# JANUS-Institute/HallThrusterPEM

Measured on AMD Instinct MI355X. Metric: coupled PEM-v0 model evals/sec, higher is better.
Workload: dtype f64

## Files before the change

### hallthrusterpem_amd/_lib.py

```python
import ctypes as C
import importlib.util
import os
import threading
from pathlib import Path

PKG = Path(__file__).resolve().parent
LIB_PATH = PKG / 'libpem_hip.so'

PEM_OK, PEM_ERR_INVALID_ARG, PEM_ERR_HIP, PEM_ERR_NO_DEVICE = 0, 1, 2, 3
NANGLE = 91
FUSED_LATENT_MAX_RANK = 8
FUSED_SYSTEM_MAX_RECORDS = 1024
SYS_JION, SYS_VCC, SYS_T, SYS_UION = 0, 1, 2, 3
SWEEP_CATHODE, SWEEP_THRUSTER, SWEEP_PLUME = 0, 1, 2
DE_MAX_POP, DE_MAX_DIM = 1024, 16
DE_BEST1BIN, DE_RAND1BIN = 0, 1
CHAIN_TIME_BLOCK = 4096

_dp = C.c_void_p
_sz = C.c_size_t
_f8 = C.c_double

SIGNATURES = {
    'pem_version': (C.c_char_p, []),
    'pem_last_error': (C.c_char_p, []),
    'pem_device_count': (C.c_int, []),
    'pem_init': (C.c_int, [C.c_int]),
    'pem_synchronize': (C.c_int, [_dp]),
    'pem_set_lanes_per_sample': (C.c_int, [C.c_int]),
    'pem_angle_grid': (C.POINTER(C.c_double), []),
    'pem_persistent_grid': (C.c_int, [_sz, C.c_int, C.c_int, C.c_int, C.POINTER(_sz), C.POINTER(_sz)]),
    'pem_coupled_occupancy': (C.c_int, [C.c_int, C.POINTER(C.c_int), C.POINTER(C.c_int)]),
    'pem_cathode_f64_dev': (C.c_int, [_sz] + [_dp] * 6 + [_f8, _dp, _dp]),
    'pem_cathode_f64': (C.c_int, [_sz] + [_dp] * 6 + [_f8, _dp]),
    'pem_plume_f64_dev': (C.c_int, [_sz, C.c_int, _dp, _f8] + [_dp] * 10 + [_dp] * 4 + [_dp]),
    'pem_plume_f64': (C.c_int, [_sz, C.c_int, _dp, _f8] + [_dp] * 10 + [_dp] * 4),
    'pem_thruster_f64_dev': (C.c_int, [_sz] + [_dp] * 4 + [_dp] * 8 + [_dp]),
    'pem_thruster_f64': (C.c_int, [_sz] + [_dp] * 4 + [_dp] * 8),
    'pem_thruster_uion_f64_dev': (C.c_int, [_sz, _dp, _f8, _f8, C.c_int, _dp, _dp, _dp]),
    'pem_thruster_filter_f64_dev': (C.c_int, [_sz, C.c_int, _dp, _dp, _f8, C.c_int, _dp, _dp, _dp, _dp]),
    'pem_coupled_f64_dev': (C.c_int, [_sz, _f8, _f8] + [_dp] * 15 + [_dp] * 7 + [_dp]),
    'pem_coupled_f64': (C.c_int, [_sz, _f8, _f8] + [_dp] * 15 + [_dp] * 7),
    'pem_coupled_tiled_f64_dev': (C.c_int, [_sz, _f8, _f8, _dp] + [_dp] * 7 + [_dp]),
    'pem_coupled_mixed_dev': (C.c_int, [_sz, _f8, _f8] + [_dp] * 15 + [_dp] * 7 + [_dp]),
    'pem_coupled_loglik_f64_dev': (C.c_int, [_sz, _f8, _f8] + [_dp] * 15 + [C.c_int, C.c_int] + [_dp] * 4 + [_dp] * 5 + [_dp]),
    'pem_coupled_system_loglik_f64_dev': (C.c_int, [_sz, _f8, _f8] + [_dp] * 15 + [C.c_int, C.c_int, _dp, _dp, C.c_int, _dp, _f8, _f8, C.c_int]
                                          + [_dp] * 5 + [_dp]),
    'pem_coupled_system_predict_f64_dev': (C.c_int, [_sz, _f8, _f8] + [_dp] * 15 + [C.c_int, C.c_int, _dp, _dp, C.c_int, _dp, _f8, _f8, C.c_int]
                                           + [_dp] * 4 + [_sz, _dp, _dp]),
    'pem_predictive_inputs_f64_dev': (C.c_int, [_sz, C.c_int, C.c_uint64, C.c_uint64, C.c_uint32, _dp, _dp, _dp, _dp, _dp, _sz, C.c_int,
                                                _dp, C.c_uint32, _dp, _sz, _dp]),
    'pem_predictive_noise_f64_dev': (C.c_int, [_sz, C.c_int, _dp, _sz, _dp, C.c_uint64, C.c_uint64, C.c_uint32, _dp, _sz, _dp]),
    'pem_coupled_latent_f64_dev': (C.c_int, [_sz, _f8, _f8] + [_dp] * 15 + [C.c_int, C.c_int, _dp, _dp] + [_dp] * 4 + [_dp]),
    'pem_loglik_marginal_f64_dev': (C.c_int, [_sz, C.c_int, C.c_int, _dp, _dp, _dp, _f8, _f8, _dp, _dp, _dp]),
    'pem_log_prior_f64_dev': (C.c_int, [_sz, C.c_int, _dp, _dp, _dp, _dp, _dp, _dp, _dp, _dp]),
    'pem_jion_loglik_f64_dev': (C.c_int, [_sz, C.c_int, C.c_int] + [_dp] * 6 + [_dp]),
    'pem_svd_compress_f64_dev': (C.c_int, [_sz, C.c_int, C.c_int, C.c_int, _f8, _dp, _dp, _dp, _dp]),
    'pem_svd_reconstruct_f64_dev': (C.c_int, [_sz, C.c_int, C.c_int, C.c_int, _f8, _dp, _dp, _dp, _dp]),
    'pem_coupled_mc_f64_dev': (C.c_int, [_sz, C.c_uint64, C.c_uint64, C.c_uint32, C.c_int, _dp, _dp, _dp, _f8, _f8, _dp, _sz] + [_dp] * 7 + [_dp]),
    'pem_sparse_predict_f64_dev': (C.c_int, [_sz, C.c_int, C.c_int, _dp, _dp, _dp, C.c_int, _dp, _sz, _dp, _sz, C.c_int, C.c_int, _dp]),
    'pem_sparse_grid_values_f64_dev': (C.c_int, [_sz, C.c_int, C.c_int, _dp, _dp, _dp, C.c_int, _dp, _sz, _dp, _sz, C.c_int, C.c_int, _dp]),
    'pem_sparse_predict_field_f64_dev': (C.c_int, [_sz, C.c_int, C.c_int, _dp, _dp, _dp, C.c_int, _dp, _sz, _dp, _sz, C.c_int, C.c_int,
                                                   C.c_int, C.c_int, C.c_int, C.c_int, C.c_double, _dp, _dp, _dp]),
    'pem_sparse_predict_chain_f64_dev': (C.c_int, [_sz, C.c_int, C.c_int, C.c_int, _dp, _f8, _f8, _f8, _f8, _dp, _sz, _dp, _sz,
                                                   C.c_int, C.c_int, C.c_int, C.c_int, C.c_double, _dp, _dp, _dp]),
    'pem_key_minmax_f64_dev': (C.c_int, [_sz, C.c_int, _dp, _sz, _dp, _dp, _dp, _dp]),
    'pem_range_hist_f64_dev': (C.c_int, [_sz, C.c_int, _dp, _sz, C.c_int, _dp, _dp, C.c_int, _dp, _dp]),
    'pem_range_narrow_dev': (C.c_int, [C.c_int, C.c_int, _dp, _dp, _dp, _dp, _dp]),
    'pem_qsel_bins': (C.c_int, [C.c_int, C.c_int, C.POINTER(C.c_int), C.POINTER(C.c_int)]),
    'pem_qsel_minmax_f64_dev': (C.c_int, [_sz, C.c_int, _dp, _sz, _dp, _dp, _dp, _dp]),
    'pem_qsel_hist1_f64_dev': (C.c_int, [_sz, C.c_int, _dp, _sz, _dp, _dp, C.c_int, _dp, _dp]),
    'pem_qsel_decide1_dev': (C.c_int, [C.c_int, C.c_int, _dp, _dp, _dp, C.c_int, _dp, _dp, _dp, _dp, _dp]),
    'pem_qsel_hist2_f64_dev': (C.c_int, [_sz, C.c_int, _dp, _sz, _dp, _dp, C.c_int, _dp, C.c_int, C.c_int, _dp, _dp]),
    'pem_qsel_decide2_dev': (C.c_int, [C.c_int, C.c_int, _dp, _dp, C.c_int, _dp, _dp, _dp, _dp, _dp, _dp, _dp]),
    'pem_qsel_compact_f64_dev': (C.c_int, [_sz, C.c_int, _dp, _sz, _dp, _dp, C.c_int, _dp, _dp, _dp, C.c_int, C.c_int, C.c_uint32, _dp, _dp, _dp]),
    'pem_qsel_select_dev': (C.c_int, [C.c_int, C.c_int, C.c_int, C.c_uint32, _dp, _dp, _dp, _dp, _dp, _dp, _dp]),
    'pem_quantiles_f64_dev': (C.c_int, [_sz, C.c_int, _dp, _sz, C.c_int, _dp, _dp, _dp, _dp, _dp]),
    'pem_quantiles_strided_f64_dev': (C.c_int, [_sz, C.c_int, _dp, _sz, _sz, C.c_int, _dp, _dp, _dp, _dp, _dp]),
    'pem_quantiles_last_path': (C.c_int, []),
    'pem_coupled_mc_stats_f64_dev': (C.c_int, [_sz, C.c_uint64, C.c_uint64, C.c_uint32, _dp, _dp, _dp, C.c_double, C.c_double, _dp, _sz,
                                               _dp, _dp, _dp, _dp, _dp, _dp, _dp, _dp, C.c_int, _dp, _dp, _dp, _dp, _dp, _dp,
                                               C.c_int, C.c_int, C.c_double, _dp, _dp, _dp, _dp]),
    'pem_row_masks_f64_dev': (C.c_int, [_sz, C.c_int, _dp, _sz, _dp, _dp, _dp, _dp, _dp]),
    'pem_campaign_masks_f64_dev': (C.c_int, [_sz, C.c_int, _dp, _dp, C.c_int, C.c_int, C.c_int, C.c_double, _dp, _dp, _sz, _dp, _dp, C.c_int, _dp, _dp,
                                             C.c_int, _dp]),
    'pem_sobol_partial_f64_dev': (C.c_int, [_sz, C.c_int, _sz, _dp, _dp, _dp, _dp, C.c_int, _dp]),
    'pem_coupled_f32_dev': (C.c_int, [_sz, C.c_float, C.c_float, _dp, _sz, _dp, _sz, _dp, _dp]),
    'pem_saltelli_f32_dev': (C.c_int, [_sz, C.c_uint64, C.c_uint64, C.c_uint32, _dp, _dp, _dp, C.c_int, _dp, C.c_float, C.c_float, _dp, _dp, C.c_int, _dp]),
    'pem_saltelli_f64_dev': (C.c_int, [_sz, C.c_uint64, C.c_uint64, C.c_uint32, _dp, _dp, _dp, C.c_int, _dp, C.c_double, C.c_double, _dp, _dp, C.c_int, _dp]),
    'pem_sobol_sweep_f64_dev': (C.c_int, [C.c_int, _sz, C.c_uint64, C.c_uint64, C.c_int, _dp, _dp, _dp, _f8, _f8, _f8, _f8, _f8, C.c_int,
                                          _dp, _dp, _dp, _dp, C.c_int, _dp]),
    'pem_de_step_f64_dev': (C.c_int, [C.c_int, C.c_int, C.c_int, C.c_int, C.c_uint64, _f8, _f8, _f8, _f8, _f8, _dp, _dp, _dp, _dp, _dp, _dp,
                                      _dp, _dp, _dp, _dp, _dp, _sz, _dp]),
    'pem_sample_f64_dev': (C.c_int, [_sz, C.c_uint64, C.c_uint64, C.c_uint32, C.c_int, _dp, _dp, _dp, C.c_int, _dp, _sz, _dp]),
    'pem_sample_tiled_f64_dev': (C.c_int, [_sz, C.c_uint64, C.c_uint64, C.c_uint32, C.c_int, _dp, _dp, _dp, C.c_int, _dp, _dp]),
    'pem_sample_lhs_f64_dev': (C.c_int, [_sz, C.c_uint64, C.c_uint64, C.c_uint64, C.c_uint32, C.c_int, _dp, _dp, _dp, _dp, _sz, _dp]),
    'pem_chain_autocov_f64_dev': (C.c_int, [_sz, _sz, _sz, _dp] + [_sz] * 6 + [_dp, _dp, _dp, _sz, _dp]),
}


class SurrStage(C.Structure):
    _fields_ = [('index', _dp), ('coef', _dp), ('values', _dp), ('n_beta', C.c_int), ('n_out', C.c_int), ('max_active', C.c_int),
                ('max_level', C.c_int)]


_lib = None
_hip_runtime = None
_lock = threading.Lock()


class PemHipError(RuntimeError):

    def __init__(self, code, message):
        super().__init__(f'libpem_hip error {code}: {message}')
        self.code = code


def _share_torch_hip_runtime():
    if os.environ.get('PEM_HIP_RUNTIME', '').lower() == 'system':
        return None
    try:
        spec = importlib.util.find_spec('torch')
    except (ImportError, ValueError):
        spec = None
    if spec is None or not spec.submodule_search_locations:
        return None
    cand = Path(list(spec.submodule_search_locations)[0]) / 'lib' / 'libamdhip64.so'
    if not cand.exists():
        return None
    return C.CDLL(str(cand), mode=C.RTLD_GLOBAL)


def load():
    global _lib, _hip_runtime
    if _lib is not None:
        return _lib
    with _lock:
        if _lib is not None:
            return _lib
        path = Path(os.environ.get('PEM_HIP_LIB', LIB_PATH))
        if 'PEM_HIP_LIB' not in os.environ:
            from . import build as _build
            if _build.needs_build():
                if _build.have_hipcc():
                    _build.build()
                elif not path.exists():
                    raise RuntimeError('libpem_hip.so is missing and hipcc is not available to build it')
                else:
                    import warnings
                    warnings.warn('libpem_hip.so is older than its sources and hipcc is not available: loading the stale library')
        _hip_runtime = _share_torch_hip_runtime()
        lib = C.CDLL(str(path))
        for name, (res, args) in SIGNATURES.items():
            fn = getattr(lib, name)
            fn.restype = res
            fn.argtypes = args
        _lib = lib
    return _lib


def check(rc: int):
    if rc != PEM_OK:
        raise PemHipError(rc, load().pem_last_error().decode(errors='replace'))


# ... 29 lines not shown
```

### hallthrusterpem_amd/csrc/pem_kernels.hip

```cpp
#include <hip/hip_runtime.h>

#include <cmath>
#include <cstdarg>
#include <cstdint>
#include <cstdio>
#include <cstdlib>
#include <cstring>
#include <atomic>
#include <functional>
#include <future>
#include <mutex>
#include <string>
#include <thread>
#include <type_traits>

#include "pem_common.h"
#include "pem_math.h"
#include "pem_hip.h"
#include "pem_philox.h"
#include "pem_qfused.h"

#include "pem_model.h"

namespace {
// ... 2204 lines not shown

template <int JMODE>
int launch_count(const PlumeIO& io, const CoupledIO& cio, const McDesign& mc, int nq, hipStream_t st, unsigned* grid_only) {
    if (io.q.premask && nq <= 5) return launch_r1<4, true, JMODE, true, 5, true>(io, cio, st, mc, grid_only);
    if (nq <= 3) return launch_r1<4, true, JMODE, true, 3>(io, cio, st, mc, grid_only);
    if (nq <= 5) return launch_r1<4, true, JMODE, true, 5>(io, cio, st, mc, grid_only);
    return launch_r1<4, true, JMODE, true, 6>(io, cio, st, mc, grid_only);
}

}

namespace pem {

int launch_coupled_mc(const McLaunch& a, hipStream_t st) {
    if (a.n == 0) return PEM_OK;
    McDesign mc{};
    if (int rc = mc_design_of(a, &mc)) return rc;
    PlumeIO io{(long long)a.n, a.torr2pa, a.radius, nullptr, nullptr, nullptr, nullptr, nullptr, nullptr, nullptr, nullptr, nullptr, nullptr, a.j_ion, a.div_angle, a.T_c, a.invalid, nullptr};
    CoupledIO cio{nullptr, nullptr, nullptr, nullptr, nullptr, nullptr, nullptr, a.V_cc, a.I_B0, a.T};
    return a.j_ion ? launch_r1<4, true, 1, true>(io, cio, st, mc) : launch_r1<4, true, 0, true>(io, cio, st, mc);
}

static int count_launch(const McLaunch& a, const CountIO& c, bool store_profile, hipStream_t st, unsigned* grid_only) {
    McDesign mc{};
    if (int rc = mc_design_of(a, &mc)) return rc;
    PlumeIO io{(long long)a.n, a.torr2pa, a.radius, nullptr, nullptr, nullptr, nullptr, nullptr, nullptr, nullptr, nullptr, nullptr, nullptr, a.j_ion, a.div_angle, a.T_c, a.invalid, nullptr};
    io.q = c;
    CoupledIO cio{nullptr, nullptr, nullptr, nullptr, nullptr, nullptr, nullptr, a.V_cc, a.I_B0, a.T};
    return store_profile ? launch_count<4>(io, cio, mc, c.nq, st, grid_only) : launch_count<5>(io, cio, mc, c.nq, st, grid_only);
}

int coupled_count_waves(size_t n, int nq, bool store_profile, unsigned* waves) {
    McLaunch a{};
    a.n = n;
    for (int d = 0; d < 15; ++d) a.kind[d] = PEM_DIST_UNIFORM;
    CountIO c{};
    c.nq = nq;
    unsigned grid = 0;
    if (int rc = count_launch(a, c, store_profile, nullptr, &grid)) return rc;
    *waves = grid * WPB;
    return PEM_OK;
}

int launch_coupled_mc_count(const McLaunch& a, const CountIO& c, bool store_profile, hipStream_t st) {
    if (a.n == 0) return PEM_OK;
    if (c.nq < 1 || c.nq > 6 || !c.br || !c.below || !c.rec || !c.rec_count || !c.flags || c.cap == 0)
        return fail(PEM_ERR_INVALID_ARG, "counting launch: incomplete arguments");
    if (store_profile && !a.j_ion) return fail(PEM_ERR_INVALID_ARG, "counting launch: no profile array to store into");
    return count_launch(a, c, store_profile, st, nullptr);
}

}

extern "C" {

namespace {
struct ScalarJob {
    struct Stage {
        std::promise<int> go;
        std::future<int> gone;
        bool signalled = false;
        hipEvent_t ev = nullptr;
        Stage() : gone(go.get_future()) {}
        void signal(int v) {
            if (!signalled) {
                signalled = true;
                go.set_value(v);
            }
        }
        int launched(hipStream_t st) {
            if (signalled) return PEM_OK;
            HIP_TRY(hipEventRecord(ev, st));
            signal(1);
            return PEM_OK;
        }
        int await(hipStream_t side) {
            if (gone.get() != 1) return fail(PEM_ERR_HIP, "pem_coupled_mc_stats (scalar selection): given up");
            HIP_TRY(hipStreamWaitEvent(side, ev, 0));
            return PEM_OK;
        }
    };
    Stage pilot, full;
    Stage side;
    std::thread worker;
    std::function<void()> body;
    bool started = false;
    int rc = PEM_OK;
    std::string error;
    int start() {
        if (started) return PEM_OK;
        started = true;
        HIP_TRY(hipEventCreateWithFlags(&pilot.ev, hipEventDisableTiming));
        HIP_TRY(hipEventCreateWithFlags(&full.ev, hipEventDisableTiming));
        HIP_TRY(hipEventCreateWithFlags(&side.ev, hipEventDisableTiming));
        try {
            worker = std::thread(body);
        } catch (const std::exception& e) {
            return fail(PEM_ERR_HIP, "pem_coupled_mc_stats: could not start the scalar selection's thread: %s", e.what());
        }
        return PEM_OK;
    }
    int join() {
        pilot.signal(0);
        full.signal(0);
        if (worker.joinable()) worker.join();
        for (Stage* s : {&pilot, &full, &side}) {
            if (s->ev) (void)hipEventDestroy(s->ev);
            s->ev = nullptr;
        }
        return rc;
    }
    ~ScalarJob() { (void)join(); }
};

int side_stream(hipStream_t* out) {
    static std::mutex mu;
    static hipStream_t streams[64] = {};
    int dev = 0;
    HIP_TRY(hipGetDevice(&dev));
    if (dev < 0 || dev >= 64) return fail(PEM_ERR_INVALID_ARG, "device index out of range");
    std::lock_guard<std::mutex> lock(mu);
    if (!streams[dev]) HIP_TRY(hipStreamCreateWithFlags(&streams[dev], hipStreamNonBlocking));
    *out = streams[dev];
    return PEM_OK;
}

struct McProducer : pem::FusedProducer {
    pem::McLaunch a;
    bool store_profile;
    bool counted = false;
    ScalarJob* job = nullptr;
    int pilot(size_t rows, double* dst, hipStream_t st) override {
        pem::McLaunch p = a;
        p.n = rows;
        p.j_ion = dst;
        if (int rc = pem::launch_coupled_mc(p, st)) return rc;
        if (!job) return PEM_OK;
        if (int rc = job->start()) return rc;
        return job->pilot.launched(st);
    }
    int waves(int nq, unsigned* w) override { return pem::coupled_count_waves(a.n, nq, store_profile, w); }
    int count(const pem::CountIO& io, hipStream_t st) override {
        if (job && job->worker.joinable() && job->side.gone.get() == 1) HIP_TRY(hipStreamWaitEvent(st, job->side.ev, 0));
        if (int rc = pem::launch_coupled_mc_count(a, io, store_profile, st)) return rc;
        counted = true;
        return job ? job->full.launched(st) : PEM_OK;
    }
};
}

int pem_coupled_mc_stats_f64_dev(size_t n, uint64_t first_index, uint64_t seed, uint32_t stream_id, const int32_t* kind, const double* a,
                                 const double* b, double torr2pa, double radius, double* x_out, size_t ld, double* V_cc, double* I_B0,
                                 double* T, double* j_ion, double* pilot_rows, double* div_angle, double* T_c, uint8_t* invalid, int nq,
                                 const uint64_t* rank_prev, const uint64_t* rank_next, const double* gamma, double* q_out, double* q_scalars,
                                 int* fused_ok, int q25, int q75, double iqr_factor, uint8_t* row_certain, uint8_t* row_uncertain,
                                 int* premask_ok, pem_stream_t stream) {
    if (!kind || !a || !b || !V_cc || !div_angle || !T_c || !rank_prev || !rank_next || !gamma || !q_out || !fused_ok)
        return fail(PEM_ERR_INVALID_ARG, "pem_coupled_mc_stats: NULL array");
    if (!j_ion && !pilot_rows) return fail(PEM_ERR_INVALID_ARG, "pem_coupled_mc_stats: without a profile array, room for the pilot rows is needed");
    if (j_ion && !aligned16(j_ion)) return fail(PEM_ERR_INVALID_ARG, "pem_coupled_mc_stats: j_ion must be 16-byte aligned");
    if (pilot_rows && !aligned16(pilot_rows)) return fail(PEM_ERR_INVALID_ARG, "pem_coupled_mc_stats: pilot_rows must be 16-byte aligned");
    if (x_out && ld < n) return fail(PEM_ERR_INVALID_ARG, "pem_coupled_mc_stats: leading dimension smaller than n");
    if (nq < 1 || nq > PEM_QUANTILE_MAX_Q) return fail(PEM_ERR_INVALID_ARG, "pem_coupled_mc_stats: 1 <= nq <= %d", PEM_QUANTILE_MAX_Q);
    if (n < PEM_MC_STATS_MIN_N) return fail(PEM_ERR_INVALID_ARG, "pem_coupled_mc_stats: at least %d samples", PEM_MC_STATS_MIN_N);
    const ptrdiff_t qstride = div_angle - V_cc;
    if (q_scalars && (qstride < (ptrdiff_t)n || T_c - div_angle != qstride))
        return fail(PEM_ERR_INVALID_ARG, "pem_coupled_mc_stats: q_scalars needs V_cc, div_angle, T_c as equally spaced rows of one array");
    if (int rc = check_device()) return rc;
    hipStream_t st = static_cast<hipStream_t>(stream);
    ScalarJob job;
    McProducer prod;
    if (q_scalars) {
        int dev = 0;
        HIP_TRY(hipGetDevice(&dev));
        hipStream_t side = nullptr;
        if (int rc = side_stream(&side)) return rc;
        job.body = [&job, dev, side, n, nq, V_cc, qstride, rank_prev, rank_next, gamma, q_scalars]() {
            struct Release {
                ScalarJob& j;
                ~Release() { j.side.signal(0); }
            } release{job};
            auto note = [&job](int rc) {
                job.rc = rc;
                if (rc != PEM_OK) job.error = pem_last_error();
                return rc;
            };
            if (hipSetDevice(dev) != hipSuccess) {
                (void)note(fail(PEM_ERR_HIP, "pem_coupled_mc_stats (scalar selection): hipSetDevice failed"));
                return;
            }
            if (note(job.pilot.await(side))) return;
            pem::SidePlan plan;
            plan.ctx = &job;
            plan.before_full = [](void* ctx, hipStream_t st) {
                ScalarJob* j = static_cast<ScalarJob*>(ctx);
                if (j->side.launched(st)) j->side.signal(0);
                return j->full.await(st);
            };
            (void)note(pem::quantiles_side(n, 3, V_cc, 1, (size_t)qstride, nq, rank_prev, rank_next, gamma, q_scalars, side, &plan));
        };
        prod.job = &job;
    }
    prod.a.n = n;
    prod.a.first_index = first_index;
    prod.a.seed = seed;
    prod.a.stream_id = stream_id;
    for (int d = 0; d < 15; ++d) {
        prod.a.kind[d] = kind[d];
        prod.a.a[d] = a[d];
        prod.a.b[d] = b[d];
    }
    prod.a.torr2pa = torr2pa;
    prod.a.radius = radius;
    prod.a.x_out = x_out;
    prod.a.ld = ld;
    prod.a.V_cc = V_cc;
    prod.a.I_B0 = I_B0;
    prod.a.T = T;
    prod.a.j_ion = j_ion;
    prod.a.div_angle = div_angle;
    prod.a.T_c = T_c;
    prod.a.invalid = invalid;
    prod.store_profile = j_ion != nullptr;
    if (row_certain && row_uncertain && premask_ok) {
        prod.pm_q25 = q25;
        prod.pm_q75 = q75;
        prod.pm_factor = iqr_factor;
        prod.pm_certain = row_certain;
        prod.pm_uncertain = row_uncertain;
    }
    if (premask_ok) *premask_ok = 0;
    *fused_ok = 0;
    if (int rc = pem::quantiles_fused(n, NANG, nq, rank_prev, rank_next, gamma, j_ion ? j_ion : pilot_rows, prod, q_out, fused_ok, st))
        return rc;
    if (premask_ok) *premask_ok = (*fused_ok && prod.pm_done) ? 1 : 0;
    if (!*fused_ok && !prod.counted) {
        if (int rc = pem::launch_coupled_mc(prod.a, st)) return rc;
        if (q_scalars) {
            if (int rc = job.start()) return rc;
            if (int rc = job.pilot.launched(st)) return rc;
            if (int rc = job.full.launched(st)) return rc;
        }
        HIP_TRY(hipStreamSynchronize(st));
    }
    if (q_scalars) {
        if (int rc = job.join()) return fail(rc, "%s", job.error.c_str());
    }
    return PEM_OK;
}

int pem_coupled_loglik_f64_dev(size_t n, double torr2pa, double radius, const double* P_b, const double* V_a,
                               const double* T_e, const double* V_vac, const double* Pstar, const double* P_T,
                               const double* mdot_a, const double* a_1, const double* c0, const double* c1, const double* c2,
                               const double* c3, const double* c4, const double* c5, const double* sigma_cex, int n_cond,
                               int n_ang, const int32_t* kidx, const double* weight, const double* y, const double* inv_std,
                               double* V_cc, double* div_angle, double* T_c, double* loglik, uint8_t* invalid,
                               pem_stream_t stream) {
    if (n_cond < 1 || n_ang < 1 || (long long)n_cond * (n_ang | 1) > PEM_FUSED_LOGLIK_MAX_MEASUREMENTS)
        return fail(PEM_ERR_INVALID_ARG, "pem_coupled_loglik: 1 <= n_cond * (n_ang | 1) <= %d", PEM_FUSED_LOGLIK_MAX_MEASUREMENTS);
    if (n == 0) return PEM_OK;
    if (!P_b || !V_a || !T_e || !V_vac || !Pstar || !P_T || !mdot_a || !a_1 || !c0 || !c1 || !c2 || !c3 || !c4 || !c5 ||
        !sigma_cex || !kidx || !weight || !y || !inv_std || !V_cc || !div_angle || !T_c || !loglik)
        return fail(PEM_ERR_INVALID_ARG, "pem_coupled_loglik: NULL array");
    if (int rc = check_device()) return rc;
    PlumeIO io{(long long)n, torr2pa, radius, P_b, c0, c1, c2, c3, c4, c5, sigma_cex, nullptr, nullptr, nullptr, div_angle, T_c, invalid, nullptr,
               kidx, weight, y, inv_std, loglik, n_cond, n_ang};
    CoupledIO cio{V_a, T_e, V_vac, Pstar, P_T, mdot_a, a_1, V_cc, nullptr, nullptr};
    return launch_r1<4, true, 3>(io, cio, static_cast<hipStream_t>(stream));
}

int pem_coupled_system_loglik_f64_dev(size_t n, double torr2pa, double radius, const double* P_b, const double* V_a,
                                      const double* T_e, const double* V_vac, const double* Pstar, const double* P_T,
                                      const double* mdot_a, const double* a_1, const double* c0, const double* c1, const double* c2,
                                      const double* c3, const double* c4, const double* c5, const double* sigma_cex, int n_cond,
                                      int n_rec, const double* rec, const int32_t* span, int n_node, const int32_t* node, double z0,
                                      double z1, int ncells, double* V_cc, double* div_angle, double* T_c, double* loglik,
                                      uint8_t* invalid, pem_stream_t stream) {
    if (n_cond < 1 || n_cond > PEM_FUSED_SYSTEM_MAX_RECORDS || n_rec < 0 || n_rec > PEM_FUSED_SYSTEM_MAX_RECORDS || n_node < 0 ||
        n_node > 2 * PEM_FUSED_SYSTEM_MAX_RECORDS)
        return fail(PEM_ERR_INVALID_ARG, "pem_coupled_system_loglik: 1 <= n_cond <= %d, 0 <= n_rec <= %d, 0 <= n_node <= %d "
                    "(PEM_FUSED_SYSTEM_MAX_RECORDS)", PEM_FUSED_SYSTEM_MAX_RECORDS, PEM_FUSED_SYSTEM_MAX_RECORDS,
                    2 * PEM_FUSED_SYSTEM_MAX_RECORDS);
    if (n_node > 0 && ncells < 2) return fail(PEM_ERR_INVALID_ARG, "pem_coupled_system_loglik: need at least 2 u_ion grid points");
    if (n == 0) return PEM_OK;
    if (!P_b || !V_a || !T_e || !V_vac || !Pstar || !P_T || !mdot_a || !a_1 || !c0 || !c1 || !c2 || !c3 || !c4 || !c5 ||
        !sigma_cex || (n_rec > 0 && !rec) || !span || (n_node > 0 && !node) || !V_cc || !div_angle || !T_c || !loglik)
        return fail(PEM_ERR_INVALID_ARG, "pem_coupled_system_loglik: NULL array");
    if (int rc = check_device()) return rc;
    PlumeIO io{(long long)n, torr2pa, radius, P_b, c0, c1, c2, c3, c4, c5, sigma_cex, nullptr, nullptr, nullptr, div_angle, T_c, invalid, nullptr,
               nullptr, nullptr, nullptr, nullptr, loglik, n_cond, 0};
    CoupledIO cio{V_a, T_e, V_vac, Pstar, P_T, mdot_a, a_1, V_cc, nullptr, nullptr};
    const SystemTable tab{rec, span, node, n_rec, n_node, z0, z1, ncells};
    return launch_r1<4, true, 6>(io, cio, static_cast<hipStream_t>(stream), McDesign{}, nullptr, &tab);
}

int pem_coupled_system_predict_f64_dev(size_t n, double torr2pa, double radius, const double* P_b, const double* V_a,
                                       const double* T_e, const double* V_vac, const double* Pstar, const double* P_T,
                                       const double* mdot_a, const double* a_1, const double* c0, const double* c1, const double* c2,
                                       const double* c3, const double* c4, const double* c5, const double* sigma_cex, int n_cond,
                                       int n_rec, const double* rec, const int32_t* span, int n_node, const int32_t* node, double z0,
                                       double z1, int ncells, double* V_cc, double* div_angle, double* T_c, double* pred,
                                       size_t ld_pred, uint8_t* invalid, pem_stream_t stream) {
    if (n_cond < 1 || n_cond > PEM_FUSED_SYSTEM_MAX_RECORDS || n_rec < 0 || n_rec > PEM_FUSED_SYSTEM_MAX_RECORDS || n_node < 0 ||
        n_node > 2 * PEM_FUSED_SYSTEM_MAX_RECORDS)
        return fail(PEM_ERR_INVALID_ARG, "pem_coupled_system_predict: 1 <= n_cond <= %d, 0 <= n_rec <= %d, 0 <= n_node <= %d "
                    "(PEM_FUSED_SYSTEM_MAX_RECORDS)", PEM_FUSED_SYSTEM_MAX_RECORDS, PEM_FUSED_SYSTEM_MAX_RECORDS,
                    2 * PEM_FUSED_SYSTEM_MAX_RECORDS);
    if (n_node > 0 && ncells < 2) return fail(PEM_ERR_INVALID_ARG, "pem_coupled_system_predict: need at least 2 u_ion grid points");
    if (ld_pred < (size_t)n_rec) return fail(PEM_ERR_INVALID_ARG, "pem_coupled_system_predict: ld_pred < n_rec");
    if (n == 0) return PEM_OK;
    if (!P_b || !V_a || !T_e || !V_vac || !Pstar || !P_T || !mdot_a || !a_1 || !c0 || !c1 || !c2 || !c3 || !c4 || !c5 ||
        !sigma_cex || (n_rec > 0 && !rec) || !span || (n_node > 0 && !node) || !pred)
        return fail(PEM_ERR_INVALID_ARG, "pem_coupled_system_predict: NULL array");
    if (int rc = check_device()) return rc;
    PlumeIO io{(long long)n, torr2pa, radius, P_b, c0, c1, c2, c3, c4, c5, sigma_cex, nullptr, nullptr, nullptr, div_angle, T_c, invalid, nullptr,
               nullptr, nullptr, nullptr, nullptr, nullptr, n_cond, 0};
    CoupledIO cio{V_a, T_e, V_vac, Pstar, P_T, mdot_a, a_1, V_cc, nullptr, nullptr};
    SystemPredict pr;
    static_cast<SystemTable&>(pr) = SystemTable{rec, span, node, n_rec, n_node, z0, z1, ncells};
    pr.pred = pred;
    pr.ld_pred = (long long)ld_pred;
    return launch_r1<4, true, 7>(io, cio, static_cast<hipStream_t>(stream), McDesign{}, nullptr, nullptr, &pr);
}

int pem_coupled_mixed_dev(size_t n, double torr2pa, double radius, const double* P_b, const double* V_a, const double* T_e,
                          const double* V_vac, const double* Pstar, const double* P_T, const double* mdot_a,
                          const double* a_1, const double* c0, const double* c1, const double* c2, const double* c3,
                          const double* c4, const double* c5, const double* sigma_cex, double* V_cc, double* I_B0,
                          double* T, float* j_ion_f32, double* div_angle, double* T_c, uint8_t* invalid,
                          pem_stream_t stream) {
    if (n == 0) return PEM_OK;
// ... 199 lines not shown
```

### hallthrusterpem_amd/csrc/pem_masks.hip

```cpp
#include <hip/hip_runtime.h>

#include <cstdint>

#include "pem_common.h"
#include "pem_hip.h"

namespace {

typedef unsigned long long u64;
constexpr int MBLOCK = 256;
constexpr int MWAVES = MBLOCK / 64;
constexpr int MROWS = 8;

__global__ __launch_bounds__(MBLOCK) void row_masks_narrow_kernel(long long n, int m, size_t ld, const double* __restrict__ data,
                                                                   const double* __restrict__ lo, const double* __restrict__ hi,
                                                                   uint8_t* __restrict__ nan_out, int32_t* __restrict__ outside_out) {
    const int lane = threadIdx.x & 63, rpw = 64 / m;
    const bool active = lane < rpw * m;
    const int c = lane % m, rsub = lane / m;
    const double l = active ? lo[c] : 0.0, h = active ? hi[c] : 0.0;
    const u64 row_bits = m == 64 ? ~0ull : ((1ull << m) - 1);
    const long long wave = (long long)blockIdx.x * MWAVES + (threadIdx.x >> 6), nwaves = (long long)gridDim.x * MWAVES;
    const long long groups = (n + rpw - 1) / rpw;
    for (long long g0 = wave * MROWS; g0 < groups; g0 += nwaves * MROWS) {
        double x[MROWS];
        bool ok[MROWS];
#pragma unroll
        for (int u = 0; u < MROWS; ++u) {
            const long long row = (g0 + u) * rpw + rsub;
            ok[u] = active && row < n;
            x[u] = ok[u] ? data[(size_t)row * ld + c] : 0.0;
        }
#pragma unroll
        for (int u = 0; u < MROWS; ++u) {
            const u64 out = __ballot(ok[u] && (x[u] < l || x[u] > h)), nan = __ballot(ok[u] && x[u] != x[u]);
            if (ok[u] && c == 0) {
                const long long row = (g0 + u) * rpw + rsub;
                outside_out[row] = __popcll((out >> lane) & row_bits);
                nan_out[row] = ((nan >> lane) & row_bits) ? 1 : 0;
            }
        }
    }
}

template <int NC, int ROWS = 16 / NC>
__global__ __launch_bounds__(MBLOCK) void row_masks_wide_kernel(long long n, int m, size_t ld, const double* __restrict__ data,
                                                                 const double* __restrict__ lo, const double* __restrict__ hi,
                                                                 uint8_t* __restrict__ nan_out, int32_t* __restrict__ outside_out) {
    const int lane = threadIdx.x & 63;
    double l[NC], h[NC];
    bool on[NC];
#pragma unroll
    for (int j = 0; j < NC; ++j) {
        const int c = lane + 64 * j;
        on[j] = c < m;
        l[j] = on[j] ? lo[c] : 0.0;
        h[j] = on[j] ? hi[c] : 0.0;
    }
    const long long wave = (long long)blockIdx.x * MWAVES + (threadIdx.x >> 6), nwaves = (long long)gridDim.x * MWAVES;
    for (long long r0 = wave * ROWS; r0 < n; r0 += nwaves * ROWS) {
        double x[ROWS][NC];
#pragma unroll
        for (int u = 0; u < ROWS; ++u) {
#pragma unroll
            for (int j = 0; j < NC; ++j) x[u][j] = (on[j] && r0 + u < n) ? data[(size_t)(r0 + u) * ld + lane + 64 * j] : 0.0;
        }
        int my_count = 0, my_nan = 0;
#pragma unroll
        for (int u = 0; u < ROWS; ++u) {
            int count = 0;
            u64 nan = 0;
#pragma unroll
            for (int j = 0; j < NC; ++j) {
                count += __popcll(__ballot(on[j] && (x[u][j] < l[j] || x[u][j] > h[j])));
                nan |= __ballot(on[j] && x[u][j] != x[u][j]);
            }
            if (lane == u) {
                my_count = count;
                my_nan = nan ? 1 : 0;
            }
        }
        if (lane < ROWS && r0 + lane < n) {
            outside_out[r0 + lane] = my_count;
            nan_out[r0 + lane] = (uint8_t)my_nan;
        }
    }
}

}

namespace {

constexpr int CM_MAX_VARS = 8;
struct CampaignVars {
    const double* v[CM_MAX_VARS];
};
template <int V>
__global__ __launch_bounds__(MBLOCK) void campaign_masks_kernel(long long n, int nvar, CampaignVars vars, const double* __restrict__ q, int q_ld,
                                                                int row25, int row75, double factor, uint8_t* __restrict__ nan_out,
                                                                uint8_t* __restrict__ outl_out, size_t mask_ld, const uint8_t* __restrict__ certain,
                                                                const uint8_t* __restrict__ uncertain, int thresh,
                                                                long long* __restrict__ open_rows, int* __restrict__ open_count, int cap) {
    double lo[CM_MAX_VARS], hi[CM_MAX_VARS];
#pragma unroll
    for (int k = 0; k < CM_MAX_VARS; ++k) {
        const double p25 = k < nvar ? q[(size_t)row25 * q_ld + k] : 0.0, p75 = k < nvar ? q[(size_t)row75 * q_ld + k] : 0.0;
        const double iqr = __dsub_rn(p75, p25);
        lo[k] = __dsub_rn(p25, __dmul_rn(factor, iqr));
        hi[k] = __dadd_rn(p75, __dmul_rn(factor, iqr));
    }
    const long long stride = (long long)gridDim.x * MBLOCK * V;
    for (long long i = ((long long)blockIdx.x * MBLOCK + threadIdx.x) * V; i < n; i += stride) {
        const int left = n - i < V ? (int)(n - i) : V;
#pragma unroll
        for (int k = 0; k < CM_MAX_VARS; ++k) {
            if (k < nvar) {
                unsigned nanw = 0, outw = 0;
#pragma unroll
                for (int u = 0; u < V; ++u) {
                    const double x = u < left ? vars.v[k][i + u] : 0.0;
                    nanw |= (unsigned)(x != x) << (8 * u);
                    outw |= (unsigned)((x < lo[k]) | (x > hi[k])) << (8 * u);
                }
                uint8_t* np_ = nan_out + (size_t)k * mask_ld + i;
                uint8_t* op_ = outl_out + (size_t)k * mask_ld + i;
                if (V == 4 && left == V) {
                    *reinterpret_cast<unsigned*>(np_) = nanw;
                    *reinterpret_cast<unsigned*>(op_) = outw;
                } else {
                    for (int u = 0; u < left; ++u) {
                        np_[u] = (uint8_t)(nanw >> (8 * u));
                        op_[u] = (uint8_t)(outw >> (8 * u));
                    }
                }
            }
        }
        if (certain) {
            unsigned outw = 0, cw = 0, uw = 0;
            if (V == 4 && left == V) {
                cw = *reinterpret_cast<const unsigned*>(certain + i);
                uw = *reinterpret_cast<const unsigned*>(uncertain + i);
            } else {
                for (int u = 0; u < left; ++u) {
                    cw |= (unsigned)certain[i + u] << (8 * u);
                    uw |= (unsigned)uncertain[i + u] << (8 * u);
                }
            }
#pragma unroll
            for (int u = 0; u < V; ++u) {
                if (u >= left) break;
                const int c = (int)((cw >> (8 * u)) & 255u), w = (int)((uw >> (8 * u)) & 255u);
                const bool out = c > thresh;
                outw |= (unsigned)out << (8 * u);
                if (!out && c + w > thresh) {
                    const int at = atomicAdd(open_count, 1);
                    if (at < cap) open_rows[at] = i + u;
                }
            }
            uint8_t* np_ = nan_out + (size_t)nvar * mask_ld + i;
            uint8_t* op_ = outl_out + (size_t)nvar * mask_ld + i;
            if (V == 4 && left == V) {
                *reinterpret_cast<unsigned*>(np_) = 0u;
                *reinterpret_cast<unsigned*>(op_) = outw;
            } else {
                for (int u = 0; u < left; ++u) {
                    np_[u] = 0;
                    op_[u] = (uint8_t)(outw >> (8 * u));
                }
            }
        }
    }
}

}

extern "C" int pem_campaign_masks_f64_dev(size_t n, int nvar, const double* const* vars, const double* q, int q_ld, int row25, int row75,
                                          double iqr_factor, uint8_t* nan_out,
                                          uint8_t* outl_out, size_t mask_ld, const uint8_t* row_certain, const uint8_t* row_uncertain, int thresh,
                                          int64_t* open_rows, int32_t* open_count, int cap, pem_stream_t stream) {
    if (nvar < 0 || nvar > CM_MAX_VARS) return pem::fail(PEM_ERR_INVALID_ARG, "pem_campaign_masks: 0 <= nvar <= %d", CM_MAX_VARS);
    if (!nan_out || !outl_out || (nvar && (!vars || !q))) return pem::fail(PEM_ERR_INVALID_ARG, "pem_campaign_masks: NULL array");
    if (nvar && (q_ld < nvar || row25 < 0 || row75 < 0)) return pem::fail(PEM_ERR_INVALID_ARG, "pem_campaign_masks: rows of q hold nvar values, q_ld apart");
    if ((row_certain != nullptr) != (row_uncertain != nullptr) || (row_certain && (!open_rows || !open_count || cap < 0)))
        return pem::fail(PEM_ERR_INVALID_ARG, "pem_campaign_masks: the premask counts come with open_rows and open_count");
    if (mask_ld < n) return pem::fail(PEM_ERR_INVALID_ARG, "pem_campaign_masks: rows of the mask arrays shorter than n");
    if (n == 0) return PEM_OK;
    if (int rc = pem::check_device()) return rc;
    CampaignVars cv{};
    for (int k = 0; k < nvar; ++k) {
        if (!vars[k]) return pem::fail(PEM_ERR_INVALID_ARG, "pem_campaign_masks: NULL variable");
        cv.v[k] = vars[k];
    }
    int cus = 0;
    HIP_TRY(pem::device_cus(&cus));
    const bool words = mask_ld % 4 == 0 && reinterpret_cast<uintptr_t>(nan_out) % 4 == 0 && reinterpret_cast<uintptr_t>(outl_out) % 4 == 0 &&
                       reinterpret_cast<uintptr_t>(row_certain) % 4 == 0 && reinterpret_cast<uintptr_t>(row_uncertain) % 4 == 0;
    const int v = words ? 4 : 1;
    long long blocks = (((long long)n + v - 1) / v + MBLOCK - 1) / MBLOCK;
    if (blocks > (long long)cus * 16) blocks = (long long)cus * 16;
    hipStream_t st = static_cast<hipStream_t>(stream);
    if (words)
        hipLaunchKernelGGL(campaign_masks_kernel<4>, dim3((unsigned)blocks), dim3(MBLOCK), 0, st, (long long)n, nvar, cv, q, q_ld, row25, row75, iqr_factor,
                           nan_out, outl_out, mask_ld, row_certain, row_uncertain, thresh, (long long*)open_rows, (int*)open_count, cap);
    else
        hipLaunchKernelGGL(campaign_masks_kernel<1>, dim3((unsigned)blocks), dim3(MBLOCK), 0, st, (long long)n, nvar, cv, q, q_ld, row25, row75, iqr_factor,
                           nan_out, outl_out, mask_ld, row_certain, row_uncertain, thresh, (long long*)open_rows, (int*)open_count, cap);
    HIP_TRY(hipGetLastError());
    return PEM_OK;
}

extern "C" int pem_row_masks_f64_dev(size_t n, int m, const double* data, size_t ld, const double* lo, const double* hi, uint8_t* nan_out,
                                     int32_t* outside_out, pem_stream_t stream) {
    if (m < 1 || m > PEM_ROW_MASKS_MAX_M) return pem::fail(PEM_ERR_INVALID_ARG, "pem_row_masks: 1 <= m <= %d entries per sample", PEM_ROW_MASKS_MAX_M);
    if (ld < (size_t)m) return pem::fail(PEM_ERR_INVALID_ARG, "pem_row_masks: leading dimension smaller than m");
    if (n == 0) return PEM_OK;
    if (!data || !lo || !hi || !nan_out || !outside_out) return pem::fail(PEM_ERR_INVALID_ARG, "pem_row_masks: NULL array");
    if (int rc = pem::check_device()) return rc;
    hipStream_t st = static_cast<hipStream_t>(stream);
    const long long rpw = m <= 64 ? 64 / m : 1, groups = ((long long)n + rpw - 1) / rpw;
    const int rows = m <= 64 ? MROWS : (m <= 128 ? 8 : (m <= 256 ? 4 : 2));
    long long blocks = (groups + (long long)MWAVES * rows - 1) / ((long long)MWAVES * rows);
    int cus = 0;
    HIP_TRY(pem::device_cus(&cus));
    const long long cap = (long long)cus * 8;
    if (blocks > cap) blocks = cap;
    const dim3 grid((unsigned)blocks), blk(MBLOCK);
    if (m <= 64)
        hipLaunchKernelGGL(row_masks_narrow_kernel, grid, blk, 0, st, (long long)n, m, ld, data, lo, hi, nan_out, outside_out);
    else if (m <= 128)
        hipLaunchKernelGGL(row_masks_wide_kernel<2>, grid, blk, 0, st, (long long)n, m, ld, data, lo, hi, nan_out, outside_out);
    else if (m <= 256)
        hipLaunchKernelGGL(row_masks_wide_kernel<4>, grid, blk, 0, st, (long long)n, m, ld, data, lo, hi, nan_out, outside_out);
    else
        hipLaunchKernelGGL(row_masks_wide_kernel<8>, grid, blk, 0, st, (long long)n, m, ld, data, lo, hi, nan_out, outside_out);
    HIP_TRY(hipGetLastError());
    return PEM_OK;
}
```

### hallthrusterpem_amd/csrc/pem_qfused.h

```cpp
#pragma once
#include <hip/hip_runtime.h>

#include <cstdint>

namespace pem {

struct Bracket {
    unsigned long long lo, hi;
    unsigned loh;
    unsigned words;
    unsigned mult;
    unsigned pad;
};

struct Record {
    unsigned long long key;
    unsigned long long col;
};

__device__ __forceinline__ unsigned long long order_key(double x) {
    const unsigned long long b = (unsigned long long)__double_as_longlong(x);
    return (b >> 63) ? ~b : (b | 0x8000000000000000ull);
}
__device__ __forceinline__ unsigned order_key_high(int high_word) {
    return (unsigned)high_word ^ ((unsigned)(high_word >> 31) | 0x80000000u);
}

struct CountIO {
    const Bracket* br = nullptr;
    int nq = 0;
    unsigned long long* below = nullptr;
    Record* rec = nullptr;
    unsigned* rec_count = nullptr;
    unsigned cap = 0;
    int* flags = nullptr;
    const uint4* premask = nullptr;
    uint8_t* row_certain = nullptr;
    uint8_t* row_uncertain = nullptr;
};

struct McLaunch {
    size_t n = 0;
    unsigned long long first_index = 0, seed = 0;
    unsigned stream_id = 0;
    int kind[15];
    double a[15], b[15];
    double torr2pa = 0, radius = 0;
    double* x_out = nullptr;
    size_t ld = 0;
    double *V_cc = nullptr, *I_B0 = nullptr, *T = nullptr, *j_ion = nullptr, *div_angle = nullptr, *T_c = nullptr;
    uint8_t* invalid = nullptr;
};

__attribute__((visibility("hidden"))) int launch_coupled_mc(const McLaunch& a, hipStream_t st);
__attribute__((visibility("hidden"))) int coupled_count_waves(size_t n, int nq, bool store_profile, unsigned* waves);
__attribute__((visibility("hidden"))) int launch_coupled_mc_count(const McLaunch& a, const CountIO& c, bool store_profile, hipStream_t st);

struct FusedProducer {
    virtual ~FusedProducer() {}
    int pm_q25 = -1, pm_q75 = -1;
    double pm_factor = 0.0;
    uint8_t *pm_certain = nullptr, *pm_uncertain = nullptr;
    int pm_done = 0;
    virtual int pilot(size_t rows, double* dst, hipStream_t st) = 0;
    virtual int waves(int nq, unsigned* waves) = 0;
    virtual int count(const CountIO& io, hipStream_t st) = 0;
};
__attribute__((visibility("hidden"))) int quantiles_fused(size_t n, int m, int nq, const uint64_t* rank_prev, const uint64_t* rank_next,
                                                          const double* gamma, double* pilot_rows, FusedProducer& prod, double* out,
                                                          int* fused_ok, hipStream_t st);
struct SidePlan {
    int (*before_full)(void* ctx, hipStream_t st) = nullptr;
    void* ctx = nullptr;
};
__attribute__((visibility("hidden"))) int quantiles_side(size_t n, int m, const double* data, size_t ld, size_t cs, int nq,
                                                         const uint64_t* rank_prev, const uint64_t* rank_next, const double* gamma, double* out,
                                                         hipStream_t st, const SidePlan* plan = nullptr);

}
```

### hallthrusterpem_amd/csrc/pem_quantile.hip

```cpp
#include <hip/hip_runtime.h>

#include <atomic>
#include <cmath>
#include <cstdint>
#include <cstdlib>
#include <mutex>

#include "pem_common.h"
#include "pem_hip.h"
#include "pem_qfused.h"

namespace {

typedef unsigned long long u64;
constexpr int QBLOCK = 512;
constexpr int QWAVES = QBLOCK / 64;
constexpr int LDS_WORDS = 36864;
constexpr int SORT_CAP = 4096;
constexpr int SORT_DIRECT = 512;
constexpr int MAX_NC = 4;
constexpr int UNROLL = 8;
static_assert(PEM_QUANTILE_MAX_Q == 6, "hist2_kernel / compact_kernel are instantiated for 2, 4, ... 12 ranks per column");

__device__ __forceinline__ u64 key_of(double x) {
    const u64 b = (u64)__double_as_longlong(x);
    return (b >> 63) ? ~b : (b | 0x8000000000000000ull);
}
__device__ __forceinline__ double value_of(u64 k) {
    const u64 b = (k >> 63) ? (k & 0x7fffffffffffffffull) : ~k;
    return __longlong_as_double((long long)b);
}
struct Scale {
    u64 lo;
    unsigned mult;
    int shift;
};
__device__ __forceinline__ int bin_of(u64 k, const Scale& s, unsigned& frac) {
    const unsigned d = (unsigned)((k - s.lo) >> s.shift);
    const u64 p = (u64)d * s.mult;
    frac = (unsigned)p;
    return (int)(p >> 32);
}
__device__ __forceinline__ int subbin_of(unsigned frac, int bins2) { return (int)__umulhi(frac, (unsigned)bins2); }
__device__ __forceinline__ void keys_of_bin(const Scale& sc, u64 kmax, int bins2, long long g, u64& klo, u64& khi) {
    const u64 D = kmax >= sc.lo ? (kmax - sc.lo) >> sc.shift : 0;
    auto first = [&](long long G) {
        u64 lo = 0, hi = D + 1;
        while (lo < hi) {
            const u64 mid = (lo + hi) >> 1, prod = mid * sc.mult;
            const long long gd = (long long)(prod >> 32) * bins2 + (bins2 > 1 ? (long long)__umulhi((unsigned)prod, (unsigned)bins2) : 0);
            if (gd >= G) hi = mid;
            else lo = mid + 1;
        }
        return lo;
    };
    const u64 d0 = first(g), d1 = first(g + 1);
    klo = sc.lo + (d0 << sc.shift);
    khi = d1 > D ? kmax : sc.lo + (d1 << sc.shift) - 1;
    if (d0 > D || d0 >= d1) {
        klo = ~0ull;
        khi = 0ull;
    }
}
__device__ __forceinline__ int bin_of_d(u64 k, u64 lo, double inv, int bins) {
    const int b = (int)((double)(k - lo) * inv);
    return b < bins - 1 ? b : bins - 1;
}

struct Column {
    u64 kmin, kmax;
    int has_nan, pad;
    unsigned mult;
    int shift;
};
struct Target {
    u64 rank;
    u64 count;
    u64 offset;
    u64 cursor;
    u64 answer;
    int bin1, bin2;
    int owner;
    int done;
};

struct Lanes {
    int rpw, active, col0, rsub;
    size_t cs = 1;
// ... 190 lines not shown
                                                      Target* __restrict__ tg, long long rows, int* __restrict__ inconsistent) {
    const int i = blockIdx.x, lane = threadIdx.x;
    const int c = i / nt;
    if (i == c * nt) {
        u64 sum = 0;
        for (int b = lane; b < bins1; b += 64) sum += hist1[(size_t)c * bins1 + b];
#pragma unroll
        for (int sh = 32; sh >= 1; sh >>= 1) sum += __shfl_xor(sum, sh);
        if (lane == 0 && sum != (u64)(rows - col[c].has_nan)) atomicExch(inconsistent, 1 + c);
    }
    Target t = tg[i];
    t.owner = i - c * nt;
    if (col[c].kmin >= col[c].kmax) {
        t.done = 1;
        t.answer = col[c].kmin;
        t.bin1 = -1;
    } else {
        const Found f = find_bin(hist1 + (size_t)c * bins1, bins1, t.rank, lane);
        t.bin1 = f.bin;
        t.rank -= f.before;
    }
    if (lane == 0) tg[i] = t;
}

template <int NC, int NT>
__global__ __launch_bounds__(QBLOCK) void hist2_kernel(long long n, int m, size_t ld, size_t cs, const double* __restrict__ data, const Column* __restrict__ col,
                                                        const Target* __restrict__ tg, int bins1, int bins2,
                                                        unsigned* __restrict__ hist2) {
    extern __shared__ unsigned lds_hist[];
    for (int i = threadIdx.x; i < m * NT * bins2; i += QBLOCK) lds_hist[i] = 0;
    __syncthreads();
    const Lanes L(m, threadIdx.x & 63, cs);
    Scale sc[NC];
    int tb[NC][NT];
#pragma unroll
    for (int j = 0; j < NC; ++j) {
        const int c = L.col0 + 64 * j;
        const bool on = L.active && c < m;
        sc[j].lo = on ? col[c].kmin : 0;
        sc[j].mult = on ? col[c].mult : 0;
        sc[j].shift = on ? col[c].shift : 0;
#pragma unroll
        for (int t = 0; t < NT; ++t) {
            int b = on ? tg[c * NT + t].bin1 : -1;
#pragma unroll
            for (int u = 0; u < t; ++u)
                if (tb[j][u] == b || (on && tg[c * NT + u].bin1 == b)) b = -1;
            tb[j][t] = b;
        }
    }
    stream_values<NC>(n, m, ld, data, L, [&](int j, int c, double x) {
        if (x == x) {
            const u64 k = key_of(x);
            unsigned frac;
            const int b = bin_of(k, sc[j], frac);
            int hit = -1;
#pragma unroll
            for (int t = 0; t < NT; ++t) hit = tb[j][t] == b ? t : hit;
            if (hit >= 0) atomicAdd(&lds_hist[(c * NT + hit) * bins2 + subbin_of(frac, bins2)], 1u);
        }
    });
    __syncthreads();
    for (int i = threadIdx.x; i < m * NT * bins2; i += QBLOCK) {
        const unsigned v = lds_hist[i];
        if (v) atomicAdd(&hist2[i], v);
    }
}

__global__ __launch_bounds__(64) void decide2_kernel(int nt, const unsigned* __restrict__ hist2, int bins2, Target* __restrict__ tg) {
    const int i = blockIdx.x, lane = threadIdx.x;
    const int c = i / nt, t = i - c * nt;
    Target T = tg[i];
    if (T.done) return;
    int first = t;
    for (int u = t - 1; u >= 0; --u)
        if (!tg[c * nt + u].done && tg[c * nt + u].bin1 == T.bin1) first = u;
    const Found f = find_bin(hist2 + (size_t)(c * nt + first) * bins2, bins2, T.rank, lane);
    T.bin2 = f.bin;
    T.rank -= f.before;
    T.count = f.count;
    if (lane == 0) tg[i] = T;
}

__global__ __launch_bounds__(64 * MAX_NC) void layout_kernel(int m, int nt, Target* __restrict__ tg, u64* __restrict__ total) {
    __shared__ u64 start[64 * MAX_NC + 1];
    constexpr int NTMAX = 2 * PEM_QUANTILE_MAX_Q;
    const int c = threadIdx.x;
    int bin1[NTMAX], bin2[NTMAX], owner[NTMAX];
    bool done[NTMAX];
    u64 count[NTMAX];
    u64 mine = 0;
    if (c < m) {
#pragma unroll
        for (int t = 0; t < NTMAX; ++t) {
            const Target& T = tg[c * nt + (t < nt ? t : 0)];
            done[t] = t >= nt || T.done != 0;
            bin1[t] = T.bin1;
            bin2[t] = T.bin2;
            count[t] = T.count;
            owner[t] = t;
        }
#pragma unroll
        for (int t = 0; t < NTMAX; ++t) {
            if (done[t]) continue;
            bool found = false;
#pragma unroll
            for (int u = 0; u < NTMAX; ++u) {
                if (u < t && !found && !done[u] && bin1[u] == bin1[t] && bin2[u] == bin2[t]) {
                    owner[t] = owner[u];
                    found = true;
                }
            }
            if (owner[t] == t) mine += count[t];
        }
    }
    start[c + 1] = mine;
    if (c == 0) start[0] = 0;
    __syncthreads();
    if (c == 0) {
        for (int k = 1; k <= 64 * MAX_NC; ++k) start[k] += start[k - 1];
        total[0] = start[m];
    }
    __syncthreads();
    if (c < m) {
        u64 off = start[c];
        u64 offs[NTMAX];
#pragma unroll
        for (int t = 0; t < NTMAX; ++t) {
            offs[t] = 0;
            if (done[t]) continue;
            if (owner[t] == t) {
                offs[t] = off;
                off += count[t];
            } else {
#pragma unroll
                for (int u = 0; u < NTMAX; ++u)
                    if (u < t && u == owner[t]) offs[t] = offs[u];
            }
            tg[c * nt + t].owner = owner[t];
            tg[c * nt + t].offset = offs[t];
        }
    }
}

template <int NC, int NT>
__global__ __launch_bounds__(QBLOCK) void compact_kernel(long long n, int m, size_t ld, size_t cs, const double* __restrict__ data, const Column* __restrict__ col,
                                                          Target* __restrict__ tg, int bins1, int bins2, u64* __restrict__ cand) {
    const Lanes L(m, threadIdx.x & 63, cs);
    Scale sc[NC];
    int tb1[NC][NT], tb2[NC][NT];
#pragma unroll
    for (int j = 0; j < NC; ++j) {
        const int c = L.col0 + 64 * j;
        const bool on = L.active && c < m;
        sc[j].lo = on ? col[c].kmin : 0;
        sc[j].mult = on ? col[c].mult : 0;
        sc[j].shift = on ? col[c].shift : 0;
#pragma unroll
        for (int t = 0; t < NT; ++t) {
            const bool own = on && !tg[c * NT + t].done && tg[c * NT + t].owner == t;
            tb1[j][t] = own ? tg[c * NT + t].bin1 : -1;
            tb2[j][t] = own ? tg[c * NT + t].bin2 : -1;
        }
    }
    stream_values<NC>(n, m, ld, data, L, [&](int j, int c, double x) {
        if (x == x) {
            const u64 k = key_of(x);
            unsigned frac;
            const int b = bin_of(k, sc[j], frac);
            const int sb = subbin_of(frac, bins2);
            int hit = -1;
#pragma unroll
            for (int t = 0; t < NT; ++t) hit = (tb1[j][t] == b && tb2[j][t] == sb) ? t : hit;
            if (hit >= 0) {
                Target& T = tg[c * NT + hit];
                cand[T.offset + atomicAdd(&T.cursor, 1ull)] = k;
            }
        }
    });
}

__device__ void block_sort(u64* s, int np2) {
    for (int k = 2; k <= np2; k <<= 1) {
        for (int j = k >> 1; j > 0; j >>= 1) {
            for (int i = threadIdx.x; i < np2; i += QBLOCK) {
                const int p = i ^ j;
                if (p > i) {
                    const u64 a = s[i], b = s[p];
                    const bool up = (i & k) == 0;
                    if ((a > b) == up) {
                        s[i] = b;
                        s[p] = a;
                    }
                }
            }
            __syncthreads();
        }
    }
}

template <class List>
__device__ u64 select_from(const List& list, u64 len, u64 rank, u64 top, int* short_list = nullptr) {
    __shared__ u64 keys[SORT_CAP];
    __shared__ unsigned hist[1024];
// ... 25 lines not shown
        lo = s_lo;
        hi = s_hi;
        const u64 inside = s_cnt;
        __syncthreads();
        if (lo >= hi) return lo;
        if (inside <= SORT_DIRECT) {
            int np2 = 1;
            while (np2 < (int)inside) np2 <<= 1;
            if (threadIdx.x == 0) s_cnt = 0;
            for (int i = threadIdx.x; i < np2; i += QBLOCK) keys[i] = ~0ull;
            __syncthreads();
            for (u64 i = threadIdx.x; i < len; i += QBLOCK) {
                const u64 k = list(i);
                if (k >= lo && k <= hi) keys[atomicAdd(&s_cnt, 1ull)] = k;
            }
            __syncthreads();
            if (short_list && threadIdx.x == 0 && s_cnt != inside) atomicExch(short_list, 1);
            block_sort(keys, np2);
            const u64 r = keys[rank < inside ? rank : inside - 1];
            __syncthreads();
            return r;
        }
        for (int i = threadIdx.x; i < 1024; i += QBLOCK) hist[i] = 0;
        __syncthreads();
        const double inv = 1024.0 / ((double)(hi - lo) + 1.0);
        for (u64 i = threadIdx.x; i < len; i += QBLOCK) {
            const u64 k = list(i);
            if (k >= lo && k <= hi) atomicAdd(&hist[bin_of_d(k, lo, inv, 1024)], 1u);
        }
        __syncthreads();
        if (threadIdx.x < 64) {
            const int lane = threadIdx.x;
            u64 mine = 0;
#pragma unroll
            for (int b = 0; b < 16; ++b) mine += hist[16 * lane + b];
            u64 incl = mine;
#pragma unroll
            for (int d = 1; d < 64; d <<= 1) {
                const u64 up = __shfl_up(incl, d);
                if (lane >= d) incl += up;
            }
            const u64 before = incl - mine;
            const bool owns = incl > rank && before <= rank;
            const u64 any = __ballot(owns);
            if (any ? owns : lane == 63) {
                u64 cum = before;
                int b = 16 * lane;
                for (; b < 16 * lane + 15; ++b) {
                    if (cum + hist[b] > rank) break;
                    cum += hist[b];
                }
                s_bin = b;
                s_rank = rank - cum;
            }
        }
        __syncthreads();
        const int keep = s_bin;
        rank = s_rank;
        if (threadIdx.x == 0) {
            s_lo = ~0ull;
            s_hi = 0;
        }
        __syncthreads();
        mn = ~0ull;
        mx = 0;
        for (u64 i = threadIdx.x; i < len; i += QBLOCK) {
            const u64 k = list(i);
            if (k >= lo && k <= hi && bin_of_d(k, lo, inv, 1024) == keep) {
                mn = k < mn ? k : mn;
                mx = k > mx ? k : mx;
            }
        }
        if (mn <= mx) {
            atomicMin(&s_lo, mn);
            atomicMax(&s_hi, mx);
        }
        __syncthreads();
        lo = s_lo;
        hi = s_hi;
        __syncthreads();
    }
}

__global__ __launch_bounds__(QBLOCK) void select_kernel(int nt, Target* __restrict__ tg, const u64* __restrict__ cand, int* __restrict__ incomplete) {
    Target& T = tg[blockIdx.x];
    if (T.done) return;
    if (threadIdx.x == 0 && T.owner == (int)(blockIdx.x % nt) && T.cursor != T.count && atomicExch(incomplete, 1) == 0) {
        u64* note = reinterpret_cast<u64*>(incomplete) + 1;
        note[0] = blockIdx.x;
        note[1] = T.cursor;
        note[2] = T.count;
    }
    const u64* list = cand + T.offset;
    const u64 answer = select_from([list](u64 i) { return list[i]; }, T.count, T.rank, ~0ull, incomplete);
    if (threadIdx.x == 0) {
        T.answer = answer;
        T.done = 1;
    }
}

__global__ void finish_kernel(int m, int nq, const Column* __restrict__ col, const Target* __restrict__ tg, Wanted w,
                              double* __restrict__ out) {
#pragma clang fp contract(off)
    const int i = blockIdx.x * blockDim.x + threadIdx.x;
    if (i >= m * nq) return;
    const int q = i / m, c = i - q * m;
    const double a = value_of(tg[c * 2 * nq + 2 * q].answer), b = value_of(tg[c * 2 * nq + 2 * q + 1].answer), t = w.gamma[q];
    const double diff = b - a;
    double r = a + diff * t;
    if (t >= 0.5) r = b - diff * (1.0 - t);
    if (col[c].has_nan || col[c].kmin > col[c].kmax) r = __builtin_nan("");
    out[(size_t)q * m + c] = r;
}

using pem::Bracket;
__global__ __launch_bounds__(64) void pilot_edges_kernel(int total, int nt, int bins2, const Column* __restrict__ col, Target* __restrict__ tg) {
    const int i = blockIdx.x * blockDim.x + threadIdx.x;
    if (i >= total) return;
    Target T = tg[i];
    if (T.done) return;
    const Column C = col[i / nt];
    Scale sc;
    sc.lo = C.kmin;
    sc.mult = C.mult;
    sc.shift = C.shift;
    u64 klo, khi;
    keys_of_bin(sc, C.kmax, bins2, (long long)T.bin1 * bins2 + T.bin2, klo, khi);
    tg[i].answer = ((i % nt) & 1) ? khi : klo;
}

struct PilotEnds {
    int open_lo[PEM_QUANTILE_MAX_Q], open_hi[PEM_QUANTILE_MAX_Q];
};

__global__ void brackets_kernel(int m, int nq, const Target* __restrict__ ptg, PilotEnds e, int bins, Bracket* __restrict__ br,
                                int* __restrict__ any_single) {
    const int i = blockIdx.x * blockDim.x + threadIdx.x;
    if (i >= m * nq) return;
    const int c = i / nq, q = i - c * nq;
    u64 lo = e.open_lo[q] ? 0ull : ptg[c * 2 * nq + 2 * q].answer;
    u64 hi = e.open_hi[q] ? ~0ull : ptg[c * 2 * nq + 2 * q + 1].answer;
    if (hi < lo) hi = lo;
    Bracket b;
    const bool single = lo == hi;
    if (!single) {
        lo &= 0xffffffff00000000ull;
        hi |= 0x00000000ffffffffull;
    }
    b.lo = lo;
    b.hi = hi;
    b.loh = (unsigned)(lo >> 32);
    b.words = (unsigned)(hi >> 32) - b.loh;
    const u64 mult = (((u64)bins) << 32) / ((u64)b.words + 1);
    b.mult = single ? 0u : (mult > 0xffffffffull ? 0xffffffffu : (unsigned)mult);
    b.pad = 0;
    br[i] = b;
    if (single) atomicExch(any_single, 1);
}

__device__ __forceinline__ unsigned key_high(double x) {
    const int bh = __double2hiint(x);
    return (unsigned)bh ^ ((unsigned)(bh >> 31) | 0x80000000u);
}
__device__ __forceinline__ u64 first_t_of_bin(unsigned mult, int b, unsigned words) {
    u64 lo = 0, hi = (u64)words + 1;
    while (lo < hi) {
        const u64 mid = (lo + hi) >> 1;
        if ((int)((mid * mult) >> 32) >= b) hi = mid;
        else lo = mid + 1;
    }
    return lo;
}

constexpr int LDS_WORDS_A = 20224;
template <int NC, int NQ>
constexpr int bracket_waves_per_simd() { return NC <= 2 ? 4 : 2; }
template <int NC, int NQ>
__global__ __launch_bounds__(QBLOCK) __attribute__((amdgpu_waves_per_eu(bracket_waves_per_simd<NC, NQ>()))) void bracket_hist_kernel(long long n, int m, size_t ld, size_t cs, const double* __restrict__ data,
                                                               const Bracket* __restrict__ br, const int* __restrict__ any_single, int bins,
                                                               Column* __restrict__ col, u64* __restrict__ below, unsigned* __restrict__ hist) {
    extern __shared__ unsigned lds_hist[];
    unsigned* lds_below = lds_hist + m * NQ * bins;
    for (int i = threadIdx.x; i < m * NQ * (bins + 1); i += QBLOCK) lds_hist[i] = 0;
    __syncthreads();
    const Lanes L(m, threadIdx.x & 63, cs);
    unsigned bloh[NC][NQ], bwords[NC][NQ], bmult[NC][NQ], nbelow[NC][NQ];
    int nan[NC];
#pragma unroll
// ... 144 lines not shown
            const u64 k = key_of(x);
#pragma unroll
            for (int q = 0; q < NQ; ++q) {
                if (kh - rloh[j][q] <= rwords[j][q]) {
                    const Bracket B = br[c * NQ + q];
                    {
                        const int b = (int)__umulhi(kh - B.loh, B.mult);
                        const Target& T0 = tg[c * NT + 2 * q];
                        const Target& T1 = tg[c * NT + 2 * q + 1];
                        const int hit = (!T0.done && T0.owner == 2 * q && T0.bin2 == b) ? 2 * q
                                        : ((!T1.done && T1.owner == 2 * q + 1 && T1.bin2 == b) ? 2 * q + 1 : -1);
                        if (hit >= 0) {
                            Target& T = tg[c * NT + hit];
                            cand[T.offset + atomicAdd(&T.cursor, 1ull)] = k;
                        }
                    }
                }
            }
        }
    });
}


__global__ void bracket_check_kernel(int m, int nq, const Bracket* __restrict__ br, int* __restrict__ unfit) {
    const int i = blockIdx.x * blockDim.x + threadIdx.x;
    if (i >= m * nq) return;
    const int c = i / nq, q = i - c * nq;
    const Bracket b = br[i];
    bool bad = b.mult == 0;
    for (int u = 0; u < nq; ++u) {
        if (u == q) continue;
        const Bracket o = br[c * nq + u];
        if ((u64)b.loh <= (u64)o.loh + o.words && (u64)o.loh <= (u64)b.loh + b.words) bad = true;
    }
    if (bad) atomicExch(unfit, 1);
}

__global__ void premask_bounds_kernel(int m, int nq, const Bracket* __restrict__ br, int q25, int q75, double f, uint4* __restrict__ thr,
                                      int* __restrict__ bad) {
#pragma clang fp contract(off)
    const int c = blockIdx.x * blockDim.x + threadIdx.x;
    if (c >= m) return;
    const double A = value_of(br[c * nq + q25].lo), B = value_of(br[c * nq + q25].hi);
    const double C = value_of(br[c * nq + q75].lo), D = value_of(br[c * nq + q75].hi);
    const double iqr_max = D - A, iqr_min = C - B;
    const double lo_min = A - f * iqr_max, lo_max = B - f * iqr_min, hi_min = C + f * iqr_min, hi_max = D + f * iqr_max;
    const double v[4] = {lo_min, lo_max, hi_min, hi_max};
    bool ok = f >= 0.0;
    for (int i = 0; i < 4; ++i) ok = ok && __builtin_isfinite(v[i]) && v[i] != 0.0;
    if (!ok) atomicExch(bad, 1);
    thr[c] = make_uint4(key_high(lo_min), key_high(lo_max), key_high(hi_min), key_high(hi_max));
}

__global__ void record_total_check_kernel(const u64* __restrict__ sums, int* __restrict__ inconsistent, const int* __restrict__ prod_flags) {
    if (threadIdx.x == 0 && sums[0] != sums[1] && !prod_flags[0] && !prod_flags[1]) atomicExch(inconsistent, -1);
}

constexpr int REC_LISTS_MAX = 64 * 2 * PEM_QUANTILE_MAX_Q;

template <int NQ>
__device__ __forceinline__ int record_list(const uint4* __restrict__ s_br, const pem::Record& e, unsigned& t, unsigned& mult, bool& none) {
    const unsigned kh = (unsigned)(e.key >> 32);
    const int c0 = (int)e.col * NQ;
    int cq = c0;
    uint4 b[NQ];
#pragma unroll
    for (int q = 0; q < NQ; ++q) b[q] = s_br[c0 + q];
    t = kh - b[0].x;
    mult = b[0].z;
    none = t > b[0].y;
#pragma unroll
    for (int q = 1; q < NQ; ++q) {
        const unsigned tq = kh - b[q].x;
        if (tq <= b[q].y) {
            cq = c0 + q;
            t = tq;
            mult = b[q].z;
            none = false;
        }
    }
    return cq;
}

constexpr int REC_UNROLL = 4;

constexpr int RBLOCK = 1024;
template <int NQ>
__global__ __launch_bounds__(RBLOCK) void record_hist_kernel(const pem::Record* __restrict__ rec, const unsigned* __restrict__ rec_count, unsigned cap,
                                                              unsigned waves, const Bracket* __restrict__ br, int lists, int bins,
                                                              unsigned* __restrict__ hist) {
    extern __shared__ unsigned lds_hist[];
    __shared__ uint4 s_br[REC_LISTS_MAX];
    for (int i = threadIdx.x; i < lists * bins; i += RBLOCK) lds_hist[i] = 0;
    for (int i = threadIdx.x; i < lists; i += RBLOCK) s_br[i] = make_uint4(br[i].loh, br[i].words, br[i].mult, 0u);
    __syncthreads();
    for (unsigned w = blockIdx.x; w < waves; w += gridDim.x) {
        const unsigned cnt = rec_count[w] < cap ? rec_count[w] : cap;
        const pem::Record* r = rec + (size_t)w * cap;
        for (unsigned i0 = threadIdx.x; i0 < cnt; i0 += RBLOCK * REC_UNROLL) {
            pem::Record e[REC_UNROLL];
#pragma unroll
            for (int u = 0; u < REC_UNROLL; ++u) e[u] = r[i0 + u * RBLOCK < cnt ? i0 + u * RBLOCK : i0];
#pragma unroll
            for (int u = 0; u < REC_UNROLL; ++u) {
                unsigned t, mult;
                bool none;
                const int cq = record_list<NQ>(s_br, e[u], t, mult, none);
                if (!none && i0 + u * RBLOCK < cnt) atomicAdd(&lds_hist[cq * bins + (int)__umulhi(t, mult)], 1u);
            }
        }
    }
    __syncthreads();
    unsigned* mine = hist + (size_t)blockIdx.x * lists * bins;
    for (int i = threadIdx.x; i < lists * bins; i += RBLOCK) mine[i] = lds_hist[i];
}

__global__ __launch_bounds__(256) void record_reduce_kernel(const unsigned* __restrict__ part, int groups, int cells, unsigned* __restrict__ hist,
                                                            const unsigned* __restrict__ rec_count, unsigned cap, unsigned waves,
                                                            u64* __restrict__ sums) {
    __shared__ unsigned s_part[4][64];
    __shared__ u64 s_tot;
    const int cx = threadIdx.x & 63, slice = threadIdx.x >> 6;
    const int i = blockIdx.x * 64 + cx;
    if (threadIdx.x == 0) s_tot = 0;
    unsigned sum = 0;
    if (i < cells) {
        int g = slice;
        for (; g + 28 < groups; g += 32) {
            unsigned v[8];
#pragma unroll
            for (int u = 0; u < 8; ++u) v[u] = part[(size_t)(g + 4 * u) * cells + i];
#pragma unroll
            for (int u = 0; u < 8; ++u) sum += v[u];
        }
        for (; g < groups; g += 4) sum += part[(size_t)g * cells + i];
    }
    s_part[slice][cx] = sum;
    __syncthreads();
    if (slice == 0) {
        const unsigned all = s_part[0][cx] + s_part[1][cx] + s_part[2][cx] + s_part[3][cx];
        if (i < cells) {
            hist[i] = all;
            atomicAdd(&s_tot, (u64)all);
        }
    }
    if (blockIdx.x == 0) {
        u64 r = 0;
        for (unsigned w = threadIdx.x; w < waves; w += 256) r += rec_count[w] < cap ? rec_count[w] : cap;
        if (r) atomicAdd(&sums[1], r);
    }
    __syncthreads();
    if (threadIdx.x == 0 && s_tot) atomicAdd(&sums[0], s_tot);
}

__global__ __launch_bounds__(64) void record_offsets_kernel(int nt, int bins, const Target* __restrict__ tg, const unsigned* __restrict__ part,
                                                             int groups, int cells, unsigned* __restrict__ woff) {
    const int i = blockIdx.x, lane = threadIdx.x, targets = gridDim.x;
    const Target T = tg[i];
    const int t = i % nt;
    const bool own = !T.done && T.owner == t;
    const int cell = (i / 2) * bins + (own ? T.bin2 : 0);
    unsigned base = 0;
    for (int g0 = 0; g0 < groups; g0 += 64) {
        const int g = g0 + lane;
        const unsigned v = (own && g < groups) ? part[(size_t)g * cells + cell] : 0u;
        unsigned incl = v;
#pragma unroll
        for (int sh = 1; sh < 64; sh <<= 1) {
            const unsigned up = __shfl_up(incl, sh);
            if (lane >= sh) incl += up;
        }
        if (g < groups) woff[(size_t)g * targets + i] = base + incl - v;
        base += __shfl(incl, 63);
    }
}

template <int NQ>
__global__ __launch_bounds__(RBLOCK) void record_compact_kernel(const pem::Record* __restrict__ rec, const unsigned* __restrict__ rec_count, unsigned cap,
                                                                 unsigned waves, const Bracket* __restrict__ br, int lists, Target* __restrict__ tg,
                                                                 const unsigned* __restrict__ woff, u64* __restrict__ cand) {
    __shared__ uint4 s_br[REC_LISTS_MAX];
    __shared__ int2 s_bin[REC_LISTS_MAX];
    __shared__ unsigned s_cur[2 * REC_LISTS_MAX];
    __shared__ u64 s_base[2 * REC_LISTS_MAX];
    const unsigned* my_off = woff + (size_t)blockIdx.x * 2 * lists;
    for (int i = threadIdx.x; i < lists; i += RBLOCK) {
        s_br[i] = make_uint4(br[i].loh, br[i].words, br[i].mult, 0u);
        const Target &T0 = tg[2 * i], &T1 = tg[2 * i + 1];
        s_bin[i] = make_int2((!T0.done && (T0.owner & 1) == 0) ? T0.bin2 : -1, (!T1.done && (T1.owner & 1) == 1) ? T1.bin2 : -1);
        s_cur[2 * i] = my_off[2 * i];
        s_cur[2 * i + 1] = my_off[2 * i + 1];
        s_base[2 * i] = T0.offset;
        s_base[2 * i + 1] = T1.offset;
    }
    __syncthreads();
    for (unsigned w = blockIdx.x; w < waves; w += gridDim.x) {
        const unsigned cnt = rec_count[w] < cap ? rec_count[w] : cap;
        const pem::Record* r = rec + (size_t)w * cap;
        for (unsigned i0 = threadIdx.x; i0 < cnt; i0 += RBLOCK * REC_UNROLL) {
            pem::Record e[REC_UNROLL];
#pragma unroll
            for (int u = 0; u < REC_UNROLL; ++u) e[u] = r[i0 + u * RBLOCK < cnt ? i0 + u * RBLOCK : i0];
#pragma unroll
            for (int u = 0; u < REC_UNROLL; ++u) {
                unsigned t, mult;
                bool none;
                const int cq = record_list<NQ>(s_br, e[u], t, mult, none);
                if (none || i0 + u * RBLOCK >= cnt) continue;
                const int bin = (int)__umulhi(t, mult);
                const int2 want = s_bin[cq];
                const int hit = want.x == bin ? 0 : (want.y == bin ? 1 : -1);
                if (hit >= 0) cand[s_base[2 * cq + hit] + atomicAdd(&s_cur[2 * cq + hit], 1u)] = e[u].key;
            }
        }
    }
    __syncthreads();
    for (int i = threadIdx.x; i < 2 * lists; i += RBLOCK) {
        const unsigned wrote = s_cur[i] - my_off[i];
        if (wrote) atomicAdd(&tg[i].cursor, (u64)wrote);
    }
}

struct RangeScale {
    u64 lo, hi;
    unsigned mult;
    int shift, identity;
};
__device__ __forceinline__ RangeScale range_scale(u64 lo, u64 hi, int bins) {
    RangeScale r;
    r.lo = lo;
    r.hi = hi;
    const u64 span = hi >= lo ? hi - lo : 0;
    int shift = 0;
    while ((span >> shift) >> 31) ++shift;
    const u64 d = span >> shift;
    r.shift = shift;
    r.identity = d < (u64)bins;
    const u64 mult = (((u64)bins) << 32) / (d + 1);
    r.mult = mult > 0xffffffffull ? 0xffffffffu : (unsigned)mult;
    return r;
}

template <int NC, int NR>
__global__ __launch_bounds__(QBLOCK) void range_hist_kernel(long long n, int m, size_t ld, const double* __restrict__ data,
                                                             const u64* __restrict__ klo, const u64* __restrict__ khi, int bins,
                                                             unsigned* __restrict__ hist) {
    extern __shared__ unsigned lds_hist[];
    for (int i = threadIdx.x; i < m * NR * bins; i += QBLOCK) lds_hist[i] = 0;
    __syncthreads();
    const Lanes L(m, threadIdx.x & 63);
    RangeScale rs[NC][NR];
#pragma unroll
    for (int j = 0; j < NC; ++j) {
        const int c = L.col0 + 64 * j;
        const bool on = L.active && c < m;
#pragma unroll
        for (int r = 0; r < NR; ++r) rs[j][r] = on ? range_scale(klo[c * NR + r], khi[c * NR + r], bins) : range_scale(1, 0, bins);
    }
    stream_values<NC, (NC >= 4 && NR >= 4) ? 2 : UNROLL>(n, m, ld, data, L, [&](int j, int c, double x) {
        if (x == x) {
            const u64 k = key_of(x);
#pragma unroll
            for (int r = 0; r < NR; ++r) {
                const RangeScale& q = rs[j][r];
                if (k >= q.lo && k <= q.hi) {
                    const unsigned d = (unsigned)((k - q.lo) >> q.shift);
                    const int b = q.identity ? (int)d : (int)(((u64)d * q.mult) >> 32);
                    atomicAdd(&lds_hist[(c * NR + r) * bins + b], 1u);
                }
            }
        }
    });
    __syncthreads();
    for (int i = threadIdx.x; i < m * NR * bins; i += QBLOCK) {
        const unsigned v = lds_hist[i];
        if (v) atomicAdd(&hist[i], v);
    }
}

__global__ __launch_bounds__(64) void range_narrow_kernel(int bins, const unsigned* __restrict__ hist, u64* __restrict__ klo,
                                                           u64* __restrict__ khi, long long* __restrict__ resid) {
    const int i = blockIdx.x, lane = threadIdx.x;
    const u64 lo = klo[i], hi = khi[i];
    if (lo >= hi) return;
    const Found f = find_bin(hist + (size_t)i * bins, bins, (u64)resid[i], lane);
    if (lane != 0) return;
    const RangeScale q = range_scale(lo, hi, bins);
    const u64 b = (u64)f.bin, two32 = 1ull << 32;
    const u64 d_lo = q.identity ? b : (b * two32 + q.mult - 1) / q.mult;
    const u64 d_hi = q.identity ? b : ((b + 1) * two32 + q.mult - 1) / q.mult - 1;
    const bool last = d_hi >= ((hi - lo) >> q.shift);
    u64 nlo = lo + (d_lo << q.shift);
    u64 nhi = last ? hi : lo + (((d_hi + 1) << q.shift) - 1);
    if (nlo < lo) nlo = lo;
    if (nhi > hi) nhi = hi;
    klo[i] = nlo;
    khi[i] = nhi;
    resid[i] -= (long long)f.before;
}

__global__ void export_minmax_kernel(const Column* __restrict__ col, int m, u64* kmin, u64* kmax, int* has_nan) {
    const int c = blockIdx.x * blockDim.x + threadIdx.x;
    if (c < m) {
        kmin[c] = col[c].kmin;
        kmax[c] = col[c].kmax;
        has_nan[c] = col[c].has_nan ? 1 : 0;
    }
}

int pow2_at_most(long long x, int cap) {
    int p = 1;
    while (2LL * p <= x && 2 * p <= cap) p <<= 1;
    return p;
}

}

static std::atomic<int> g_last_path{0};
extern "C" int pem_quantiles_last_path(void) { return g_last_path.load(); }

namespace {
struct QWork {
    std::mutex mu;
    char* ws_buf = nullptr;
    size_t ws_cap = 0, cand_cap = 0, rec_cap = 0;
    u64* cand_buf = nullptr;
    pem::Record* rec_buf = nullptr;
    unsigned* part_buf = nullptr;
    size_t part_cap = 0;
    int ws_dev = -1;
};
QWork g_qwork[2];
}

static int quantiles_impl(size_t n, int m, const double* data, size_t ld, size_t cs, int nq, const uint64_t* rank_prev,
                          const uint64_t* rank_next, const double* gamma, double* out, pem_stream_t stream, pem::FusedProducer* fused,
                          int* fused_ok, int slot = 0, const pem::SidePlan* plan = nullptr) {
    if (m < 1 || m > 64 * MAX_NC) return pem::fail(PEM_ERR_INVALID_ARG, "pem_quantiles: 1 <= m <= %d columns", 64 * MAX_NC);
    if (fused && (m > 128 || !fused_ok)) return pem::fail(PEM_ERR_INVALID_ARG, "pem_quantiles: the fused form takes up to 128 columns");
    if (cs < 1 || (cs == 1 ? ld < (size_t)m : (ld != 1 || cs < n)))
        return pem::fail(PEM_ERR_INVALID_ARG, "pem_quantiles: rows of m columns (column stride 1, ld >= m) or columns of n rows (ld 1, column stride >= n)");
    if (nq < 1 || nq > (m <= 128 ? PEM_QUANTILE_MAX_Q : PEM_QUANTILE_MAX_Q_WIDE))
        return pem::fail(PEM_ERR_INVALID_ARG, "pem_quantiles: 1 <= nq <= %d per call (%d for more than 128 columns)", PEM_QUANTILE_MAX_Q, PEM_QUANTILE_MAX_Q_WIDE);
    if (n == 0) return pem::fail(PEM_ERR_INVALID_ARG, "pem_quantiles: no samples");
    if (!data || !rank_prev || !rank_next || !gamma || !out) return pem::fail(PEM_ERR_INVALID_ARG, "pem_quantiles: NULL array");
    for (int q = 0; q < nq; ++q)
        if (rank_prev[q] >= n || rank_next[q] >= n || rank_prev[q] > rank_next[q])
            return pem::fail(PEM_ERR_INVALID_ARG, "pem_quantiles: ranks must satisfy prev <= next < n");
    if (int rc = pem::check_device()) return rc;
    hipStream_t st = static_cast<hipStream_t>(stream);
    const int nt = 2 * nq;
    const int bins1 = pow2_at_most(LDS_WORDS / m, 4096), bins2 = pow2_at_most(LDS_WORDS / (m * nt), 4096);
    int binsA = pow2_at_most((m <= 128 ? LDS_WORDS_A : LDS_WORDS) / (m * nq) - 1, 4096);
    if (fused) binsA = pow2_at_most(LDS_WORDS / (m * nq), 4096);
    if (const char* e = getenv("PEM_QUANTILE_BINSA")) binsA = pow2_at_most(atoll(e) < binsA ? atoll(e) : binsA, 4096);

    long long pilot = 32, pilot_min = 1 << 25;
    if (const char* e = getenv("PEM_QUANTILE_PILOT")) pilot = atoll(e);
    if (const char* e = getenv("PEM_QUANTILE_PILOT_MIN")) pilot_min = atoll(e);
    if (fused) {
        pilot = 32;
        if (const char* e = getenv("PEM_FUSED_PILOT")) pilot = atoll(e) >= 32 ? atoll(e) : 32;
    }
    if (plan) pilot = 32;
    const bool use_pilot = fused ? true : plan ? (long long)n >= 4 * pilot : (pilot >= 2 && (long long)n * m >= pilot_min && (long long)n >= 4 * pilot);
    if (fused && (long long)n < 4 * pilot) return pem::fail(PEM_ERR_INVALID_ARG, "pem_quantiles: the fused form needs at least %lld rows", 4 * pilot);

    const size_t b_col = sizeof(Column) * m, b_tg = sizeof(Target) * m * nt;
    const size_t b_h1 = sizeof(unsigned) * (size_t)m * bins1, b_h2 = sizeof(unsigned) * (size_t)m * nt * bins2;
    const size_t b_br = sizeof(Bracket) * m * nq, b_bl = sizeof(u64) * m * nq, b_hA = sizeof(unsigned) * (size_t)m * nq * binsA;
    auto up = [](size_t x) { return (x + 255) & ~(size_t)255; };
    const size_t o_tg = up(b_col), o_h1 = o_tg + up(b_tg), o_h2 = o_h1 + up(b_h1), o_tot = o_h2 + up(b_h2);
    unsigned fused_waves = 0;
    if (fused)
        if (int rc = fused->waves(nq, &fused_waves)) return rc;
    const size_t b_rc = sizeof(unsigned) * fused_waves;
    const size_t o_br = o_tot + 256, o_bl = o_br + up(b_br), o_hA = o_bl + up(b_bl), o_rc = o_hA + up(b_hA), o_pm = o_rc + up(b_rc);
    const size_t o_end = o_pm + up(sizeof(uint4) * (size_t)m);
    QWork& work = g_qwork[slot];
    std::lock_guard<std::mutex> lock(work.mu);
    char*& ws_buf = work.ws_buf;
    size_t &ws_cap = work.ws_cap, &cand_cap = work.cand_cap, &rec_cap = work.rec_cap, &part_cap = work.part_cap;
    u64*& cand_buf = work.cand_buf;
    pem::Record*& rec_buf = work.rec_buf;
    unsigned*& part_buf = work.part_buf;
    int& ws_dev = work.ws_dev;
    int dev = 0;
    HIP_TRY(hipGetDevice(&dev));
    if (dev != ws_dev || ws_cap < o_end) {
        if (ws_buf) (void)hipFree(ws_buf);
        if (cand_buf && dev != ws_dev) {
            (void)hipFree(cand_buf);
            cand_buf = nullptr;
            cand_cap = 0;
        }
        if (rec_buf && dev != ws_dev) {
            (void)hipFree(rec_buf);
            rec_buf = nullptr;
            rec_cap = 0;
        }
        if (part_buf && dev != ws_dev) {
            (void)hipFree(part_buf);
            part_buf = nullptr;
            part_cap = 0;
        }
        ws_buf = nullptr;
        ws_cap = 0;
        HIP_TRY(hipMalloc(&ws_buf, o_end));
        ws_cap = o_end;
        ws_dev = dev;
    }
    char* ws = ws_buf;
    Column* col = reinterpret_cast<Column*>(ws);
    Target* tg = reinterpret_cast<Target*>(ws + o_tg);
    unsigned* hist1 = reinterpret_cast<unsigned*>(ws + o_h1);
    unsigned* hist2 = reinterpret_cast<unsigned*>(ws + o_h2);
    u64* total = reinterpret_cast<u64*>(ws + o_tot);
    int* outside = reinterpret_cast<int*>(total + 1);
    int* incomplete = reinterpret_cast<int*>(total + 2);
    int* any_single = reinterpret_cast<int*>(total + 8);
    int* unfit = reinterpret_cast<int*>(total + 9);
    int* prod_flags = unfit + 1;
    unsigned* rec_count = reinterpret_cast<unsigned*>(ws + o_rc);
    uint4* pm_thr = reinterpret_cast<uint4*>(ws + o_pm);
    int* pm_bad = unfit + 3;
    int* inconsistent = unfit + 4;
    Bracket* br = reinterpret_cast<Bracket*>(ws + o_br);
    u64* below = reinterpret_cast<u64*>(ws + o_bl);
    unsigned* histA = reinterpret_cast<unsigned*>(ws + o_hA);
    auto cleanup = [&](int code) {
        (void)hipStreamSynchronize(st);
        return code;
    };
#define Q_TRY(expr)                                                                                          \
    do {                                                                                                     \
        hipError_t e_ = (expr);                                                                              \
        if (e_ != hipSuccess) return cleanup(pem::fail(PEM_ERR_HIP, "%s: %s", #expr, hipGetErrorString(e_))); \
    } while (0)

    Wanted w{};
    for (int q = 0; q < nq; ++q) {
        w.prev[q] = rank_prev[q];
        w.next[q] = rank_next[q];
        w.gamma[q] = gamma[q];
    }
    const int cblocks = (m + 63) / 64;
    const int nc = m <= 64 ? 1 : (m <= 128 ? 2 : 4);
    const size_t lds1 = (size_t)m * bins1 * 4, lds2 = (size_t)m * nt * bins2 * 4, ldsA = (size_t)m * nq * (binsA + 1) * 4;
    const dim3 blk(QBLOCK);
    auto grid_for = [&](size_t rows) {
        const long long rpw = m <= 64 ? 64 / m : 1, groups = ((long long)rows + rpw - 1) / rpw;
        long long blocks = (groups + (long long)QWAVES * UNROLL - 1) / ((long long)QWAVES * UNROLL);
        if (blocks > 256 * 2) blocks = 256 * 2;
        return dim3((unsigned)blocks);
    };
    auto grow_candidates = [&](u64 need) -> hipError_t {
        if (cand_cap >= need + 1) return hipSuccess;
        if (cand_buf) (void)hipFree(cand_buf);
        cand_buf = nullptr;
        cand_cap = 0;
        const u64 room = need + need / 4 + 1024;
        const hipError_t e = hipMalloc(&cand_buf, (size_t)room * sizeof(u64));
        if (e == hipSuccess) cand_cap = room;
        return e;
    };
#define Q_LDS(KERN) (void)hipFuncSetAttribute(reinterpret_cast<const void*>(KERN), hipFuncAttributeMaxDynamicSharedMemorySize, 160 * 1024)
#define Q_BY_NC(CALL)              \
    do {                           \
        if (nc == 1) { CALL(1); }  \
        else if (nc == 2) { CALL(2); } \
        else { CALL(4); }          \
    } while (0)
#define Q_BY_NT_SMALL(CALL, NC_)       \
    do {                               \
        if (nt == 2) { CALL(NC_, 2); } \
        else if (nt == 4) { CALL(NC_, 4); } \
        else { CALL(NC_, 6); }         \
    } while (0)
#define Q_BY_NT_ALL(CALL, NC_)         \
    do {                               \
        if (nt == 2) { CALL(NC_, 2); } \
        else if (nt == 4) { CALL(NC_, 4); } \
        else if (nt == 6) { CALL(NC_, 6); } \
        else if (nt == 8) { CALL(NC_, 8); } \
        else if (nt == 10) { CALL(NC_, 10); } \
        else { CALL(NC_, 12); }        \
    } while (0)
#define Q_BY_NQ_SMALL(CALL, NC_)       \
    do {                               \
        if (nq == 1) { CALL(NC_, 1); } \
        else if (nq == 2) { CALL(NC_, 2); } \
        else { CALL(NC_, 3); }         \
    } while (0)
#define Q_BY_NQ_ALL(CALL, NC_)         \
    do {                               \
        if (nq == 1) { CALL(NC_, 1); } \
        else if (nq == 2) { CALL(NC_, 2); } \
        else if (nq == 3) { CALL(NC_, 3); } \
        else if (nq == 4) { CALL(NC_, 4); } \
        else if (nq == 5) { CALL(NC_, 5); } \
        else { CALL(NC_, 6); }         \
    } while (0)
#define Q_BY_NT_1 Q_BY_NT_ALL
#define Q_BY_NT_2 Q_BY_NT_ALL
#define Q_BY_NT_4 Q_BY_NT_SMALL
#define Q_BY_NQ_1 Q_BY_NQ_ALL
#define Q_BY_NQ_2 Q_BY_NQ_ALL
#define Q_BY_NQ_4 Q_BY_NQ_SMALL

    auto four_passes = [&](size_t rows, size_t ldd, const Wanted& ww, bool edges = false) -> int {
        const dim3 grid = grid_for(rows);
        Q_TRY(hipMemsetAsync(hist1, 0, o_tot + 256 - o_h1, st));
        hipLaunchKernelGGL(init_columns_kernel, dim3(cblocks), dim3(64), 0, st, col, tg, m, nq, ww);
#define Q_MINMAX(NC_) hipLaunchKernelGGL(minmax_kernel<NC_>, grid, blk, 0, st, (long long)rows, m, ldd, cs, data, col)
        Q_BY_NC(Q_MINMAX);
        hipLaunchKernelGGL(scale_columns_kernel, dim3(cblocks), dim3(64), 0, st, col, m, bins1);
#define Q_HIST1(NC_)                                                                                       \
    Q_LDS(hist1_kernel<NC_>);                                                                              \
    hipLaunchKernelGGL(hist1_kernel<NC_>, grid, blk, lds1, st, (long long)rows, m, ldd, cs, data, col, bins1, hist1)
        Q_BY_NC(Q_HIST1);
        hipLaunchKernelGGL(decide1_kernel, dim3((unsigned)(m * nt)), dim3(64), 0, st, m, nt, col, hist1, bins1, tg, (long long)rows, inconsistent);
#define Q_HIST2_(NC_, NT_)                                                                                                  \
    Q_LDS((hist2_kernel<NC_, NT_>));                                                                                        \
    hipLaunchKernelGGL((hist2_kernel<NC_, NT_>), grid, blk, lds2, st, (long long)rows, m, ldd, cs, data, col, tg, bins1, bins2, hist2)
#define Q_HIST2(NC_) Q_BY_NT_##NC_(Q_HIST2_, NC_)
        Q_BY_NC(Q_HIST2);
        hipLaunchKernelGGL(decide2_kernel, dim3((unsigned)(m * nt)), dim3(64), 0, st, nt, hist2, bins2, tg);
        if (edges) {
            hipLaunchKernelGGL(pilot_edges_kernel, dim3((unsigned)((m * nt + 63) / 64)), dim3(64), 0, st, m * nt, nt, bins2, col, tg);
            Q_TRY(hipGetLastError());
            return PEM_OK;
        }
        hipLaunchKernelGGL(layout_kernel, dim3(1), dim3(64 * MAX_NC), 0, st, m, nt, tg, total);
        Q_TRY(hipGetLastError());
        u64 h_total = 0;
        Q_TRY(hipMemcpyAsync(&h_total, total, sizeof(u64), hipMemcpyDeviceToHost, st));
        Q_TRY(hipStreamSynchronize(st));
        Q_TRY(grow_candidates(h_total));
        u64* cand = cand_buf;
#define Q_COMPACT_(NC_, NT_) \
    hipLaunchKernelGGL((compact_kernel<NC_, NT_>), grid, blk, 0, st, (long long)rows, m, ldd, cs, data, col, tg, bins1, bins2, cand)
#define Q_COMPACT(NC_) Q_BY_NT_##NC_(Q_COMPACT_, NC_)
        Q_BY_NC(Q_COMPACT);
        hipLaunchKernelGGL(select_kernel, dim3((unsigned)(m * nt)), blk, 0, st, nt, tg, cand, incomplete);
        Q_TRY(hipGetLastError());
        return PEM_OK;
    };

    int path = 0;
    bool answered = false;
    if (plan && !use_pilot && plan->before_full)
        if (int rc = plan->before_full(plan->ctx, st)) return cleanup(rc);
    if (use_pilot) {
        const size_t rows_p = (n + (size_t)pilot - 1) / (size_t)pilot;
        Wanted pw{};
        PilotEnds ends{};
        const double n1 = n > 1 ? (double)(n - 1) : 1.0, np1 = (double)(rows_p - 1);
        for (int q = 0; q < nq; ++q) {
            const double p_lo = (double)rank_prev[q] / n1, p_hi = (double)rank_next[q] / n1;
            double sig = fused ? 5.0 : 7.0;
            if (fused)
                if (const char* e = getenv("PEM_FUSED_SIGMA")) sig = atof(e) >= 3.0 ? atof(e) : 3.0;
            const double d_lo = sig * sqrt((double)rows_p * p_lo * (1.0 - p_lo)) + 8.0, d_hi = sig * sqrt((double)rows_p * p_hi * (1.0 - p_hi)) + 8.0;
            const double r_lo = floor(p_lo * np1 - d_lo) - 1.0, r_hi = ceil(p_hi * np1 + d_hi) + 1.0;
            ends.open_lo[q] = r_lo < 0.0;
            ends.open_hi[q] = r_hi > np1;
            pw.prev[q] = ends.open_lo[q] ? 0 : (u64)r_lo;
            pw.next[q] = ends.open_hi[q] ? (u64)(rows_p - 1) : (u64)r_hi;
        }
        if (fused) {
            if (int rc = fused->pilot(rows_p, const_cast<double*>(data), st)) return cleanup(rc);
            const bool edges = !(getenv("PEM_FUSED_PILOT_EXACT") && atoi(getenv("PEM_FUSED_PILOT_EXACT")));
            if (int rc = four_passes(rows_p, ld, pw, edges)) return rc;
        } else if (plan) {
            if (int rc = four_passes(rows_p, ld, pw)) return rc;
            if (plan->before_full)
                if (int rc = plan->before_full(plan->ctx, st)) return cleanup(rc);
        } else if (int rc = four_passes(rows_p, ld * (size_t)pilot, pw)) return rc;
        const dim3 grid = grid_for(n);
        Q_TRY(hipMemsetAsync(total, 0, 256, st));
        Q_TRY(hipMemsetAsync(below, 0, o_end - o_bl, st));
        hipLaunchKernelGGL(brackets_kernel, dim3((unsigned)((m * nq + 63) / 64)), dim3(64), 0, st, m, nq, tg, ends, binsA, br, any_single);
        hipLaunchKernelGGL(init_columns_kernel, dim3(cblocks), dim3(64), 0, st, col, tg, m, nq, w);
#define Q_BRHIST_(NC_, NQ_)                                                                                                  \
    Q_LDS((bracket_hist_kernel<NC_, NQ_>));                                                                                  \
    hipLaunchKernelGGL((bracket_hist_kernel<NC_, NQ_>), grid, blk, ldsA, st, (long long)n, m, ld, cs, data, br, any_single, binsA, col, below, histA)
#define Q_BRHIST(NC_) Q_BY_NQ_##NC_(Q_BRHIST_, NC_)
        unsigned rcap = 0;
        bool pm_launched = false;
        if (!fused) {
            Q_BY_NC(Q_BRHIST);
        } else {
            hipLaunchKernelGGL(bracket_check_kernel, dim3((unsigned)((m * nq + 63) / 64)), dim3(64), 0, st, m, nq, br, unfit);
            const bool want_pm = fused->pm_q25 >= 0 && fused->pm_q25 < nq && fused->pm_q75 >= 0 && fused->pm_q75 < nq && nq <= 5 &&
                                 fused->pm_certain && fused->pm_uncertain;
            fused->pm_done = 0;
            if (want_pm)
                hipLaunchKernelGGL(premask_bounds_kernel, dim3((unsigned)((m + 63) / 64)), dim3(64), 0, st, m, nq, br, fused->pm_q25, fused->pm_q75,
                                   fused->pm_factor, pm_thr, pm_bad);
            const bool use_pm = want_pm;
            pm_launched = want_pm;
            double expected = 0.0;
            for (int q = 0; q < nq; ++q) expected += (double)(pw.next[q] - pw.prev[q] + 1) * (double)pilot * (double)m;
            rcap = (unsigned)(1.5 * expected / (double)fused_waves) + 4096u;
            if (const char* e = getenv("PEM_QUANTILE_RECORD_CAP")) rcap = (unsigned)atoll(e);
            const size_t need = (size_t)fused_waves * rcap;
            if (rec_cap < need) {
                if (rec_buf) (void)hipFree(rec_buf);
                rec_buf = nullptr;
                rec_cap = 0;
                Q_TRY(hipMalloc(&rec_buf, need * sizeof(pem::Record)));
                rec_cap = need;
            }
            pem::CountIO cio;
            cio.br = br;
            cio.nq = nq;
            cio.below = reinterpret_cast<unsigned long long*>(below);
            cio.rec = rec_buf;
            cio.rec_count = rec_count;
            cio.cap = rcap;
            cio.flags = prod_flags;
            if (use_pm) {
                cio.premask = pm_thr;
                cio.row_certain = fused->pm_certain;
                cio.row_uncertain = fused->pm_uncertain;
            }
            if (int rc = fused->count(cio, st)) return cleanup(rc);
            int cus = 256;
            Q_TRY(pem::device_cus(&cus));
            const int cells = m * nq * binsA;
            {
                const size_t need = (size_t)cus * cells + (size_t)cus * m * nt;
                if (part_cap < need) {
                    if (part_buf) (void)hipFree(part_buf);
                    part_buf = nullptr;
                    part_cap = 0;
                    Q_TRY(hipMalloc(&part_buf, need * sizeof(unsigned)));
                    part_cap = need;
                }
            }
#define Q_RECHIST(NQ_)                                                                                                       \
    do {                                                                                                                     \
        static pem::LdsAttrOnce attr;                                                                                        \
        Q_TRY(attr.ensure(reinterpret_cast<const void*>(record_hist_kernel<NQ_>), 148 * 1024));  \
        hipLaunchKernelGGL(record_hist_kernel<NQ_>, dim3((unsigned)cus), dim3(RBLOCK), (size_t)m * nq * binsA * 4, st, rec_buf, rec_count, rcap, fused_waves, \
                           br, m * nq, binsA, part_buf);                                                                     \
    } while (0)
            switch (nq) {
                case 1: Q_RECHIST(1); break;
                case 2: Q_RECHIST(2); break;
                case 3: Q_RECHIST(3); break;
                case 4: Q_RECHIST(4); break;
                case 5: Q_RECHIST(5); break;
                default: Q_RECHIST(6); break;
            }
#undef Q_RECHIST
            u64* rec_sums = total + 16;
            hipLaunchKernelGGL(record_reduce_kernel, dim3((unsigned)((cells + 63) / 64)), dim3(256), 0, st, part_buf, cus, cells, histA, rec_count, rcap,
                               fused_waves, rec_sums);
            hipLaunchKernelGGL(record_total_check_kernel, dim3(1), dim3(64), 0, st, rec_sums, inconsistent, prod_flags);
        }
        hipLaunchKernelGGL(decide_bracket_kernel, dim3((unsigned)(m * nt)), dim3(64), 0, st, nt, col, br, below, histA, binsA, tg, outside);
        hipLaunchKernelGGL(layout_kernel, dim3(1), dim3(64 * MAX_NC), 0, st, m, nt, tg, total);
        Q_TRY(hipGetLastError());
        u64 h_tot[2] = {0, 0};
        int h_unfit4[4] = {0, 0, 0, 0};
        Q_TRY(hipMemcpyAsync(h_tot, total, 2 * sizeof(u64), hipMemcpyDeviceToHost, st));
        if (fused) Q_TRY(hipMemcpyAsync(h_unfit4, unfit, sizeof h_unfit4, hipMemcpyDeviceToHost, st));
        Q_TRY(hipStreamSynchronize(st));
        if (fused) fused->pm_done = (pm_launched && h_unfit4[3] == 0) ? 1 : 0;
        if (fused && (h_unfit4[0] || (int)(h_tot[1] & 0xffffffffull) != 0 || h_unfit4[1] || h_unfit4[2])) {
            *fused_ok = 0;
            return cleanup(PEM_OK);
        }
        if ((int)(h_tot[1] & 0xffffffffull) == 0) {
            Q_TRY(grow_candidates(h_tot[0]));
            u64* cand = cand_buf;
#define Q_BRCOMPACT_(NC_, NQ_) \
    hipLaunchKernelGGL((compact_bracket_kernel<NC_, NQ_>), grid, blk, 0, st, (long long)n, m, ld, cs, data, br, tg, cand)
#define Q_BRCOMPACT(NC_) Q_BY_NQ_##NC_(Q_BRCOMPACT_, NC_)
            if (!fused) {
                Q_BY_NC(Q_BRCOMPACT);
            } else {
                int cus = 256;
                Q_TRY(pem::device_cus(&cus));
                unsigned* woff = part_buf + (size_t)cus * m * nq * binsA;
                hipLaunchKernelGGL(record_offsets_kernel, dim3((unsigned)(m * nt)), dim3(64), 0, st, nt, binsA, tg, part_buf, cus, m * nq * binsA, woff);
#define Q_RECCOMPACT(NQ_) \
    hipLaunchKernelGGL(record_compact_kernel<NQ_>, dim3((unsigned)cus), dim3(RBLOCK), 0, st, rec_buf, rec_count, rcap, fused_waves, br, m * nq, tg, woff, cand)
                switch (nq) {
                    case 1: Q_RECCOMPACT(1); break;
                    case 2: Q_RECCOMPACT(2); break;
                    case 3: Q_RECCOMPACT(3); break;
                    case 4: Q_RECCOMPACT(4); break;
                    case 5: Q_RECCOMPACT(5); break;
                    default: Q_RECCOMPACT(6); break;
                }
#undef Q_RECCOMPACT
            }
            hipLaunchKernelGGL(select_kernel, dim3((unsigned)(m * nt)), blk, 0, st, nt, tg, cand, incomplete);
            Q_TRY(hipGetLastError());
            answered = true;
            path = 1;
        } else {
            path = 2;
        }
    }
    if (!answered)
        if (int rc = four_passes(n, ld, w)) return rc;
    hipLaunchKernelGGL(finish_kernel, dim3((unsigned)((m * nq + 63) / 64)), dim3(64), 0, st, m, nq, col, tg, w, out);
    Q_TRY(hipGetLastError());
    u64 h_incomplete[4] = {0, 0, 0, 0};
    int h_inconsistent = 0;
    Q_TRY(hipMemcpyAsync(h_incomplete, incomplete, sizeof h_incomplete, hipMemcpyDeviceToHost, st));
    Q_TRY(hipMemcpyAsync(&h_inconsistent, inconsistent, sizeof(int), hipMemcpyDeviceToHost, st));
    Q_TRY(hipStreamSynchronize(st));
    if (h_inconsistent > 0)
        return pem::fail(PEM_ERR_HIP, "pem_quantiles: the histogram of column %d does not add up to its number of values (internal error; result discarded; path %d)",
                         h_inconsistent - 1, path);
    if (h_inconsistent < 0)
        return pem::fail(PEM_ERR_HIP, "pem_quantiles: the record histogram does not add up to the number of records (internal error; result discarded)");
    if ((h_incomplete[0] & 0xffffffffull) && h_incomplete[2] == h_incomplete[3])
        return pem::fail(PEM_ERR_HIP, "pem_quantiles: a candidate list was sorted with fewer keys than it holds (internal error; result discarded; path %d)", path);
    if (h_incomplete[0] & 0xffffffffull)
        return pem::fail(PEM_ERR_HIP,
                         "pem_quantiles: the list of column %llu, rank %llu holds %llu values where %llu were counted (internal error; result "
                         "discarded; path %d)",
                         h_incomplete[1] / nt, h_incomplete[1] % nt, h_incomplete[2], h_incomplete[3], path);
    if (slot == 0) g_last_path.store(path);
    if (fused_ok) *fused_ok = 1;
#undef Q_BRCOMPACT
#undef Q_BRCOMPACT_
#undef Q_BRHIST
#undef Q_BRHIST_
#undef Q_COMPACT
#undef Q_COMPACT_
#undef Q_HIST2
#undef Q_HIST2_
#undef Q_HIST1
#undef Q_MINMAX
#undef Q_BY_NQ_4
#undef Q_BY_NQ_2
#undef Q_BY_NQ_1
#undef Q_BY_NT_4
#undef Q_BY_NT_2
#undef Q_BY_NT_1
#undef Q_BY_NQ_ALL
#undef Q_BY_NQ_SMALL
#undef Q_BY_NT_ALL
#undef Q_BY_NT_SMALL
#undef Q_BY_NC
#undef Q_LDS
#undef Q_TRY
    return cleanup(PEM_OK);
}

extern "C" int pem_quantiles_strided_f64_dev(size_t n, int m, const double* data, size_t ld, size_t cs, int nq, const uint64_t* rank_prev,
                                             const uint64_t* rank_next, const double* gamma, double* out, pem_stream_t stream) {
    return quantiles_impl(n, m, data, ld, cs, nq, rank_prev, rank_next, gamma, out, stream, nullptr, nullptr);
}

int pem::quantiles_fused(size_t n, int m, int nq, const uint64_t* rank_prev, const uint64_t* rank_next, const double* gamma, double* pilot_rows,
                         pem::FusedProducer& prod, double* out, int* fused_ok, hipStream_t st) {
    return quantiles_impl(n, m, pilot_rows, (size_t)m, 1, nq, rank_prev, rank_next, gamma, out, static_cast<pem_stream_t>(st), &prod, fused_ok);
}

int pem::quantiles_side(size_t n, int m, const double* data, size_t ld, size_t cs, int nq, const uint64_t* rank_prev, const uint64_t* rank_next,
                        const double* gamma, double* out, hipStream_t st, const pem::SidePlan* plan) {
    return quantiles_impl(n, m, data, ld, cs, nq, rank_prev, rank_next, gamma, out, static_cast<pem_stream_t>(st), nullptr, nullptr, 1, plan);
}

extern "C" int pem_quantiles_f64_dev(size_t n, int m, const double* data, size_t ld, int nq, const uint64_t* rank_prev, const uint64_t* rank_next,
                                     const double* gamma, double* out, pem_stream_t stream) {
    if (ld < (size_t)(m > 0 ? m : 0)) return pem::fail(PEM_ERR_INVALID_ARG, "pem_quantiles: leading dimension smaller than m");
    return pem_quantiles_strided_f64_dev(n, m, data, ld, 1, nq, rank_prev, rank_next, gamma, out, stream);
}

namespace {

dim3 stream_grid(size_t n, int m) {
    const long long rpw = m <= 64 ? 64 / m : 1, groups = ((long long)n + rpw - 1) / rpw;
    long long blocks = (groups + (long long)QWAVES * UNROLL - 1) / ((long long)QWAVES * UNROLL);
    if (blocks > 256 * 2) blocks = 256 * 2;
    if (blocks < 1) blocks = 1;
    return dim3((unsigned)blocks);
}

}

extern "C" int pem_key_minmax_f64_dev(size_t n, int m, const double* data, size_t ld, uint64_t* kmin, uint64_t* kmax, int32_t* has_nan,
                                      pem_stream_t stream) {
    if (m < 1 || m > 64 * MAX_NC) return pem::fail(PEM_ERR_INVALID_ARG, "pem_key_minmax: 1 <= m <= %d columns", 64 * MAX_NC);
    if (ld < (size_t)m) return pem::fail(PEM_ERR_INVALID_ARG, "pem_key_minmax: leading dimension smaller than m");
    if (!kmin || !kmax || !has_nan || (n && !data)) return pem::fail(PEM_ERR_INVALID_ARG, "pem_key_minmax: NULL array");
    if (int rc = pem::check_device()) return rc;
    hipStream_t st = static_cast<hipStream_t>(stream);
    Column* col = nullptr;
    HIP_TRY(hipMalloc(&col, sizeof(Column) * m));
    Target* no_targets = nullptr;
// ... 514 lines not shown
```

### hallthrusterpem_amd/drivers.py

```python
import functools

import numpy as np

from . import sampling
from .batch import QOI_NAMES, CoupledBatch
from .distributed import shard_bounds

COORDS_STR_ID = '_coords'


MAX_Q, MAX_Q_WIDE = 6, 3


def _linear_ranks(n: int, percentiles):
    return _linear_ranks_cached(int(n), tuple(float(x) for x in np.atleast_1d(np.asarray(percentiles, dtype=np.float64))))


@functools.lru_cache(maxsize=64)
def _linear_ranks_cached(n: int, percentiles: tuple):
    q = np.true_divide(np.asarray(percentiles, dtype=np.float64), np.float64(100))
    if not np.all((q >= 0) & (q <= 1)):
        raise ValueError('Percentiles must be in the range [0, 100]')
    if n == 0:
        raise ValueError('no samples')
# ... 151 lines not shown
        if method == 'mc':
            batch.run_mc(design, first_index=lo + off, write_inputs=keep_inputs, first=off, count=m, stream=st)
        else:
            design.fill(batch.inputs[:, off:off + m], first_index=lo + off, method=method, n_total=n, stream=st)
            batch.run(first=off, count=m, stream=st)
    if side:
        for st in side:
            caller.wait_event(st.record_event())
    out = {k: batch.qoi[i] for i, k in enumerate(QOI_NAMES)}
    out.update(I_B0=batch.I_B0, T=batch.T, invalid=batch.invalid.bool())
    if keep_inputs or method != 'mc':
        out['x'] = batch.inputs
    if keep_profile:
        out['j_ion'] = batch.j_ion
    return out


def percentile_bands(outputs: dict, percentiles=(5.0, 50.0, 95.0), names=('V_cc', 'div_angle', 'T_c', 'j_ion'), group=None,
                     sharded: bool = False):
    import torch
    if not sharded:
        return {k: column_percentiles(outputs[k], list(percentiles)) for k in names if k in outputs}
    _check_sharded_call({k: outputs[k] for k in names if k in outputs}, group)
    from .percentiles import column_percentiles_sharded
    return {k: torch.from_numpy(np.ascontiguousarray(column_percentiles_sharded(outputs[k], list(percentiles), group=group))).to(outputs[k].device)
            for k in names if k in outputs}


def _stacked_rows(tensors):
    import torch
    t0 = tensors[0]
    if len(tensors) < 2 or any(t.dim() != 1 or not t.is_cuda or t.dtype != torch.float64 or t.numel() != t0.numel() or t.stride(0) != 1
                               or t.untyped_storage().data_ptr() != t0.untyped_storage().data_ptr() for t in tensors):
        return None
    n, step = t0.numel(), tensors[1].storage_offset() - t0.storage_offset()
    if step < n or any(t.storage_offset() != t0.storage_offset() + i * step for i, t in enumerate(tensors)):
        return None
    return torch.as_strided(t0, (n, len(tensors)), (1, step))


def campaign_statistics(outputs: dict, iqr_factor: float = 1.5, percentiles=(5.0, 50.0, 95.0), names=None):
    import torch
    names = [k for k in (outputs if names is None else names) if k in outputs and COORDS_STR_ID not in str(k) and str(k) != 'errors']
    pct = [25.0, 75.0] + [float(x) for x in percentiles]
    q = {}
    scalars = [k for k in names if outputs[k].dim() == 1]
    stacked = _stacked_rows([outputs[k] for k in scalars]) if len(scalars) > 1 else None
    if stacked is not None:
        qs = column_percentiles(stacked, pct)
        q.update({k: qs[:, i] for i, k in enumerate(scalars)})
    for k in names:
        if k not in q:
            q[k] = column_percentiles(outputs[k], pct)
    nan_idx, outlier_idx, bands = {}, {}, {}
    for k in names:
        a, qk = outputs[k].double(), q[k]
        per_sample = int(np.prod(a.shape[1:])) if a.dim() > 1 else 1
        iqr = qk[1] - qk[0]
        lo, hi = qk[0] - iqr_factor * iqr, qk[1] + iqr_factor * iqr
        if a.shape[0] > 0 and per_sample <= ROW_MASKS_MAX_M:
            nan_idx[k], count = _row_masks(a, lo, hi, per_sample)
        else:
            rest = tuple(range(1, a.dim()))
            nan_idx[k] = torch.isnan(a).any(dim=rest) if rest else torch.isnan(a)
            outside = (a < lo) | (a > hi)
            count = outside.sum(dim=rest) if rest else outside.long()
        outlier_idx[k] = count > int(0.75 * per_sample)
        bands[k] = qk[2:]
    return nan_idx, outlier_idx, bands


FUSED_STATS_MIN_N = 4096


def forward_uq_statistics(n: int, seed: int = 0, keep_profile: bool = True, percentiles=(5.0, 50.0, 95.0), iqr_factor: float = 1.5,
                          priors=None, device=None, keep_inputs: bool = False, fused: bool = True):
    import ctypes as C
    import torch
    from . import _lib, constants
    design = sampling.Design(priors=priors, seed=seed)
    batch = CoupledBatch(n, device=device, profile=keep_profile)
    pct = [25.0, 75.0] + [float(x) for x in percentiles]
    answered, premasked, qj, qs, certain, uncertain = False, False, None, None, None, None
    thresh = int(0.75 * _lib.NANGLE)
    nv, cap = len(QOI_NAMES), 65536
    dev = batch.device
    with torch.cuda.device(dev):
        stream = torch.cuda.current_stream(dev)
        n_pad = (n + 3) // 4 * 4
        nan_s = torch.empty((nv + 1, n_pad), dtype=torch.bool, device=dev)[:, :n]
        out_s = torch.empty((nv + 1, n_pad), dtype=torch.bool, device=dev)[:, :n]
        open_rows = torch.empty(cap, dtype=torch.int64, device=dev)
        open_count = torch.zeros(1, dtype=torch.int32, device=dev)
        if fused and n >= FUSED_STATS_MIN_N:
            if len(pct) > MAX_Q:
                raise ValueError(f'the fused campaign takes at most {MAX_Q - 2} percentiles besides the quartiles')
            rp, rn, gm = _linear_ranks(n, pct)
            qj = torch.empty((len(pct), _lib.NANGLE), dtype=torch.float64, device=dev)
            qs = torch.empty((len(pct), nv), dtype=torch.float64, device=dev)
            pilot = None if keep_profile else torch.empty(((n + 31) // 32, _lib.NANGLE), dtype=torch.float64, device=dev)
            certain = torch.empty(n, dtype=torch.uint8, device=dev)
            uncertain = torch.empty(n, dtype=torch.uint8, device=dev)
            ok, pm_ok = C.c_int(0), C.c_int(0)
            ptr = lambda arr: C.c_void_p(arr.ctypes.data)
            outs = batch._out_ptrs
            _lib.check(_lib.load().pem_coupled_mc_stats_f64_dev(
                n, 0, design.seed, design.stream, ptr(design.kind), ptr(design.a), ptr(design.b), constants.TORR_2_PA, batch.radius,
                C.c_void_p(batch.inputs.data_ptr()) if keep_inputs else None, batch.inputs.stride(0),
                outs[0], outs[1], outs[2], outs[3], None if pilot is None else C.c_void_p(pilot.data_ptr()), outs[4], outs[5], outs[6],
                len(pct), ptr(rp), ptr(rn), ptr(gm), C.c_void_p(qj.data_ptr()), C.c_void_p(qs.data_ptr()), C.byref(ok),
                0, 1, float(iqr_factor), C.c_void_p(certain.data_ptr()), C.c_void_p(uncertain.data_ptr()), C.byref(pm_ok),
                C.c_void_p(stream.cuda_stream)))
            answered, premasked = bool(ok.value), bool(pm_ok.value)
            del pilot
        else:
            batch.run_mc(design, first_index=0, write_inputs=keep_inputs)
    out = {k: batch.qoi[i] for i, k in enumerate(QOI_NAMES)}
    out.update(I_B0=batch.I_B0, T=batch.T, invalid=batch.invalid.view(torch.bool))
    if keep_inputs:
        out['x'] = batch.inputs
    if keep_profile:
        out['j_ion'] = batch.j_ion
    full = None
    if not answered:
        if keep_profile:
            qj = column_percentiles(batch.j_ion, pct)
        else:
            full = CoupledBatch(n, device=device, profile=True, thruster_qoi=False)
            full.run_mc(design, first_index=0)
            qj = column_percentiles(full.j_ion, pct)
    if qs is None:
        qs = column_percentiles(batch.qoi.T, pct)
    q = {k: qs[:, i] for i, k in enumerate(QOI_NAMES)}
    q['j_ion'] = qj
    nan_idx, outlier_idx, bands = {}, {}, {}
    dp = lambda t: C.c_void_p(t.data_ptr())
    with torch.cuda.device(dev):
        vars_ = (C.c_void_p * nv)(*[batch.qoi[i].data_ptr() for i in range(nv)])
        _lib.check(_lib.load().pem_campaign_masks_f64_dev(
            n, nv, vars_, dp(qs), qs.stride(0), 0, 1, float(iqr_factor), dp(nan_s), dp(out_s), nan_s.stride(0), dp(certain) if premasked else None,
            dp(uncertain) if premasked else None, thresh, dp(open_rows), dp(open_count), cap, C.c_void_p(torch.cuda.current_stream(dev).cuda_stream)))
    for i, k in enumerate(QOI_NAMES):
        nan_idx[k], outlier_idx[k] = nan_s[i], out_s[i]

    def profile_bounds():
        iqr = qj[1] - qj[0]
        return qj[0] - iqr_factor * iqr, qj[1] + iqr_factor * iqr
    if premasked:
        n_open = int(open_count.item())
        if n_open > cap:
            c, u = certain.to(torch.int32), uncertain.to(torch.int32)
            rows_open = torch.nonzero((c <= thresh) & (c + u > thresh)).flatten()
        else:
            rows_open = open_rows[:n_open]
        outl = out_s[nv]
        if rows_open.numel():
            lo, hi = profile_bounds()
            rows = batch.j_ion[rows_open] if keep_profile else _profile_rows(design, rows_open, device=dev)
            outl[rows_open] = ((rows < lo) | (rows > hi)).sum(dim=1) > thresh
        nan_idx['j_ion'] = nan_s[nv]
        outlier_idx['j_ion'] = outl
    else:
        lo, hi = profile_bounds()
        prof = batch.j_ion if keep_profile else (full.j_ion if full is not None else None)
        if prof is None:
            full = CoupledBatch(n, device=device, profile=True, thruster_qoi=False)
            full.run_mc(design, first_index=0)
            prof = full.j_ion
        nan_idx['j_ion'], count = _row_masks(prof, lo, hi, _lib.NANGLE)
        outlier_idx['j_ion'] = count > thresh
    del full
    for k in q:
        bands[k] = q[k][2:]
    out.update(nan_idx=nan_idx, outlier_idx=outlier_idx, bands=bands, fused=answered, premasked=premasked)
    return out


def _profile_rows(design, indices, device=None):
    import torch
    rows = []
    one = CoupledBatch(2, device=device, profile=True, thruster_qoi=False)
    for i in indices.tolist():
        one.run_mc(design, first_index=int(i), count=1)
        rows.append(one.j_ion[0].clone())
    return torch.stack(rows)


def generate_data(system, description: str, num_samples: int = 500, executor=None, verbose: bool = False,
                  iqr_factor: float = 1.5, device_resident: bool = False):
    import os
    import pickle
    from .system import COORDS_STR_ID, to_model_dataset
    if getattr(system, 'logger', None) is not None:
        system.logger.info(f'Generating {description} data for {system.name} -- {num_samples} samples...')
    if system.root_dir is not None and not device_resident:
        os.mkdir(system.root_dir / description)
    samples = system.sample_inputs(num_samples, normalize=True, use_pdf=['calibration', 'nuisance'],
                                   as_tensor=device_resident)
    outputs = system.predict(samples, use_model='best', model_dir=None if system.root_dir is None else
                             system.root_dir / description, executor=executor, verbose=verbose)
    if device_resident:
        outputs = {k: v for k, v in outputs.items() if not k.endswith(COORDS_STR_ID)}
    samples, coords = to_model_dataset(samples, system.inputs())
    samples.update(coords)
    norm_outputs = {var.name: var.normalize(outputs[var.name]) for var in system.outputs() if var in outputs}
    nan_idx, outlier_idx = filter_outputs(norm_outputs, iqr_factor=iqr_factor)
    dump = {description: (samples, outputs), 'nan_idx': nan_idx, 'outlier_idx': outlier_idx, 'iqr_factor': iqr_factor}
    if system.root_dir is not None and not device_resident:
        with open(system.root_dir / description / f'{description}.pkl', 'wb') as fd:
            pickle.dump(dump, fd)
    return dump


def process_compression(system, data: dict, discard_outliers: bool = False):
    from .system import COORDS_STR_ID
    outputs = data['compression'][1]
    discard = discard_mask(data['nan_idx'], data['outlier_idx'], discard_outliers=discard_outliers)
    keep = ~discard
    for var in system.outputs():
        if var.compression is None:
            continue
        coords = outputs.get(f'{var}{COORDS_STR_ID}')
        if coords is not None:
            var.compression.coords = coords[0]
        if var.compression.method.lower() != 'svd':
            raise ValueError(f"Compression method '{var.compression.method}' not supported.")
        var.compression.compute_map({f: var.normalize(outputs[f][keep]) for f in var.compression.fields})
    if system.root_dir is not None:
        (system.root_dir / 'compression').mkdir(exist_ok=True)
        system.save_to_file(f'{system.name}_compression.pkl', system.root_dir / 'compression')
    return system

# ... 251 lines not shown
```

### include/pem_hip.h

```cpp
#ifndef PEM_HIP_H
#define PEM_HIP_H

#include <stddef.h>
#include <stdint.h>

#ifdef __cplusplus
extern "C" {
#endif

#define PEM_NANGLE 91

#define PEM_OK 0
#define PEM_ERR_INVALID_ARG 1
#define PEM_ERR_HIP 2
#define PEM_ERR_NO_DEVICE 3

typedef void* pem_stream_t;

const char* pem_version(void);
const char* pem_last_error(void);
int pem_device_count(void);
int pem_init(int device);
int pem_synchronize(pem_stream_t stream);
int pem_set_lanes_per_sample(int lanes);
// ... 98 lines not shown
#define PEM_SYS_JION 0
#define PEM_SYS_VCC 1
#define PEM_SYS_T 2
#define PEM_SYS_UION 3
int pem_coupled_system_loglik_f64_dev(size_t n, double torr2pa, double radius, const double* P_b, const double* V_a,
                                      const double* T_e, const double* V_vac, const double* Pstar, const double* P_T,
                                      const double* mdot_a, const double* a_1, const double* c0, const double* c1,
                                      const double* c2, const double* c3, const double* c4, const double* c5,
                                      const double* sigma_cex, int n_cond, int n_rec, const double* rec, const int32_t* span,
                                      int n_node, const int32_t* node, double z0, double z1, int ncells, double* V_cc,
                                      double* div_angle, double* T_c, double* loglik, uint8_t* invalid, pem_stream_t stream);

int pem_coupled_system_predict_f64_dev(size_t n, double torr2pa, double radius, const double* P_b, const double* V_a,
                                       const double* T_e, const double* V_vac, const double* Pstar, const double* P_T,
                                       const double* mdot_a, const double* a_1, const double* c0, const double* c1,
                                       const double* c2, const double* c3, const double* c4, const double* c5,
                                       const double* sigma_cex, int n_cond, int n_rec, const double* rec, const int32_t* span,
                                       int n_node, const int32_t* node, double z0, double z1, int ncells, double* V_cc,
                                       double* div_angle, double* T_c, double* pred, size_t ld_pred, uint8_t* invalid,
                                       pem_stream_t stream);

#define PEM_FUSED_LATENT_MAX_RANK 8
int pem_coupled_latent_f64_dev(size_t n, double torr2pa, double radius, const double* P_b, const double* V_a,
                               const double* T_e, const double* V_vac, const double* Pstar, const double* P_T,
                               const double* mdot_a, const double* a_1, const double* c0, const double* c1,
                               const double* c2, const double* c3, const double* c4, const double* c5,
                               const double* sigma_cex, int rank, int norm, const double* basis, double* latent,
                               double* V_cc, double* div_angle, double* T_c, uint8_t* invalid, pem_stream_t stream);

int pem_loglik_marginal_f64_dev(size_t n_chains, int n_draws, int n_cond, const double* loglik, const double* mdot_a,
                                const double* a_1, double discharge_current, double discharge_sigma,
                                const double* log_prior, double* out, pem_stream_t stream);
int pem_log_prior_f64_dev(size_t n, int ndim, const int32_t* kind, const double* a, const double* b, const double* lo,
                          const double* hi, const double* theta, double* out, pem_stream_t stream);

#define PEM_SVD_MAX_DOF 208
#define PEM_NORM_NONE 0
#define PEM_NORM_LOG10 1
#define PEM_NORM_LINEAR 2
int pem_svd_compress_f64_dev(size_t n, int dof, int rank, int norm, double norm_scale, const double* field,
                             const double* basis, double* latent, pem_stream_t stream);
int pem_svd_reconstruct_f64_dev(size_t n, int dof, int rank, int norm, double norm_scale, const double* latent,
                                const double* basis, double* field, pem_stream_t stream);

#define PEM_SURR_MAX_ACTIVE 5
#define PEM_SURR_MAX_LEVEL 4
#define PEM_SURR_MAX_DIM 32
int pem_sparse_predict_f64_dev(size_t n, int n_dim, int n_beta, const int32_t* index, const double* coef,
                               const double* values, int n_out, const double* t, size_t ld, double* out,
                               size_t ld_out, int max_active, int max_level, pem_stream_t stream);
int pem_sparse_grid_values_f64_dev(size_t n, int n_dim, int n_beta, const int32_t* index, const double* coef,
                                   const double* values, int n_out, const double* t, size_t ld, double* out,
                                   size_t ld_out, int max_active, int max_level, pem_stream_t stream);
int pem_sparse_predict_field_f64_dev(size_t n, int n_dim, int n_beta, const int32_t* index, const double* coef, const double* values,
                                     int n_out, const double* t, size_t ld, double* out, size_t ld_out, int max_active, int max_level,
                                     int lat0, int rank, int dof, int norm, double norm_scale, const double* basis, double* field,
                                     pem_stream_t stream);
typedef struct pem_surr_stage {
    const int32_t* index;
    const double* coef;
    const double* values;
    int n_beta, n_out, max_active, max_level;
} pem_surr_stage;
int pem_sparse_predict_chain_f64_dev(size_t n, int n_dim, int vcc_slot, int ib0_slot, const pem_surr_stage* stages, double vcc_lo,
                                     double vcc_w, double ib0_lo, double ib0_w, const double* t, size_t ld, double* out, size_t ld_out,
                                     int lat0, int rank, int dof, int norm, double norm_scale, const double* basis, double* field,
                                     pem_stream_t stream);

#define PEM_QUANTILE_MAX_Q 6
#define PEM_QUANTILE_MAX_Q_WIDE 3
int pem_quantiles_f64_dev(size_t n, int m, const double* data, size_t ld, int nq, const uint64_t* rank_prev, const uint64_t* rank_next,
                          const double* gamma, double* out, pem_stream_t stream);
int pem_quantiles_strided_f64_dev(size_t n, int m, const double* data, size_t ld, size_t cs, int nq, const uint64_t* rank_prev,
                                  const uint64_t* rank_next, const double* gamma, double* out, pem_stream_t stream);
int pem_quantiles_last_path(void);

#define PEM_MC_STATS_MIN_N 4096
int pem_coupled_mc_stats_f64_dev(size_t n, uint64_t first_index, uint64_t seed, uint32_t stream_id, const int32_t* kind, const double* a,
                                 const double* b, double torr2pa, double radius, double* x_out, size_t ld, double* V_cc, double* I_B0,
                                 double* T, double* j_ion, double* pilot_rows, double* div_angle, double* T_c, uint8_t* invalid, int nq,
                                 const uint64_t* rank_prev, const uint64_t* rank_next, const double* gamma, double* q_out, double* q_scalars,
                                 int* fused_ok, int q25, int q75, double iqr_factor, uint8_t* row_certain, uint8_t* row_uncertain,
                                 int* premask_ok, pem_stream_t stream);

#define PEM_ROW_MASKS_MAX_M 512
int pem_row_masks_f64_dev(size_t n, int m, const double* data, size_t ld, const double* lo, const double* hi, uint8_t* nan_out,
                          int32_t* outside_out, pem_stream_t stream);

int pem_campaign_masks_f64_dev(size_t n, int nvar, const double* const* vars, const double* q, int q_ld, int row25, int row75,
                               double iqr_factor, uint8_t* nan_out,
                               uint8_t* outl_out, size_t mask_ld, const uint8_t* row_certain, const uint8_t* row_uncertain, int thresh,
                               int64_t* open_rows, int32_t* open_count, int cap, pem_stream_t stream);

int pem_key_minmax_f64_dev(size_t n, int m, const double* data, size_t ld, uint64_t* kmin, uint64_t* kmax, int32_t* has_nan,
                           pem_stream_t stream);
int pem_range_hist_f64_dev(size_t n, int m, const double* data, size_t ld, int nr, const uint64_t* klo, const uint64_t* khi,
                           int bins, uint32_t* hist, pem_stream_t stream);
int pem_range_narrow_dev(int n_ranges, int bins, const uint32_t* hist, uint64_t* klo, uint64_t* khi, int64_t* resid,
                         pem_stream_t stream);

int pem_qsel_bins(int m, int nt, int* bins1, int* bins2);
int pem_qsel_minmax_f64_dev(size_t n, int m, const double* data, size_t ld, uint64_t* kmin, uint64_t* kmax, int32_t* has_nan,
                            pem_stream_t stream);
int pem_qsel_hist1_f64_dev(size_t n, int m, const double* data, size_t ld, const uint64_t* kmin, const uint64_t* kmax, int bins1,
                           uint32_t* hist1, pem_stream_t stream);
int pem_qsel_decide1_dev(int m, int nt, const uint64_t* kmin, const uint64_t* kmax, const uint32_t* hist1, int bins1, uint64_t* resid,
                         int32_t* bin1, int32_t* done, uint64_t* answer, pem_stream_t stream);
int pem_qsel_hist2_f64_dev(size_t n, int m, const double* data, size_t ld, const uint64_t* kmin, const uint64_t* kmax, int nt,
                           const int32_t* bin1, int bins1, int bins2, uint32_t* hist2, pem_stream_t stream);
int pem_qsel_decide2_dev(int m, int nt, const uint32_t* hist2, const uint32_t* hist2_local, int bins2, const int32_t* bin1,
                         const int32_t* done, uint64_t* resid, int32_t* bin2, uint64_t* count, uint32_t* count_local, pem_stream_t stream);
int pem_qsel_compact_f64_dev(size_t n, int m, const double* data, size_t ld, const uint64_t* kmin, const uint64_t* kmax, int nt,
                             const int32_t* bin1, const int32_t* bin2, const int32_t* done, int bins1, int bins2, uint32_t list_len,
                             uint64_t* cand, uint32_t* cursor, pem_stream_t stream);
int pem_qsel_select_dev(int m, int nt, int world, uint32_t list_len, const uint64_t* gathered, const int32_t* bin1, const int32_t* bin2,
                        const int32_t* done, const uint64_t* resid, uint64_t* answer, pem_stream_t stream);

int pem_coupled_mc_f64_dev(size_t n, uint64_t first_index, uint64_t seed, uint32_t stream_id, int swap_dim,
                           const int32_t* kind, const double* a, const double* b, double torr2pa, double radius,
                           double* x_out, size_t ld,
                           double* V_cc, double* I_B0, double* T, double* j_ion, double* div_angle, double* T_c,
                           uint8_t* invalid, pem_stream_t stream);

int pem_coupled_f32_dev(size_t n, float torr2pa, float radius, const float* x, size_t ld, float* qoi, size_t ldq,
                        uint8_t* invalid, pem_stream_t stream);
int pem_saltelli_f32_dev(size_t n_base, uint64_t first_index, uint64_t seed, uint32_t stream_id, const int32_t* kind,
                         const double* a, const double* b, int n_varied, const int32_t* varied, float torr2pa,
                         float radius, double* partial, uint64_t* flags, int n_blocks, pem_stream_t stream);
int pem_saltelli_f64_dev(size_t n_base, uint64_t first_index, uint64_t seed, uint32_t stream_id, const int32_t* kind,
                         const double* a, const double* b, int n_varied, const int32_t* varied, double torr2pa,
                         double radius, double* partial, uint64_t* flags, int n_blocks, pem_stream_t stream);

#define PEM_SWEEP_CATHODE 0
#define PEM_SWEEP_THRUSTER 1
#define PEM_SWEEP_PLUME 2
#define PEM_SWEEP_MAX_PRESSURES 65535
int pem_sobol_sweep_f64_dev(int group, size_t n_base, uint64_t first_index, uint64_t seed, int n_p, const int32_t* kind,
                            const double* a, const double* b, double torr2pa, double radius, double i_b0, double uion_z,
                            double spike_threshold, int max_attempts, const double* clip, double* j0_out, double* partial,
                            uint64_t* flags, int n_blocks, pem_stream_t stream);

#define PEM_DE_MAX_POP 1024
#define PEM_DE_MAX_DIM 16
#define PEM_DE_BEST1BIN 0
#define PEM_DE_RAND1BIN 1
int pem_de_step_f64_dev(int pop, int ndim, int strategy, int finalize, uint64_t seed, double mut_lo, double mut_hi, double cr,
                        double tol, double atol, const int32_t* kind, const double* a, const double* b, double* pop_u,
                        double* pop_f, double* trial_u, const double* trial_f, double* theta, uint64_t* state, double* record,
                        double* history, size_t history_len, pem_stream_t stream);

#define PEM_CHAIN_TIME_BLOCK 4096
int pem_chain_autocov_f64_dev(size_t n_rows, size_t n_series, size_t ld, const double* x, size_t n_seg, size_t seg_len,
                              size_t seg_stride, size_t lag0, size_t lag_step, size_t n_lags, double* mean, double* acov,
                              double* work, size_t work_len, pem_stream_t stream);

#ifdef __cplusplus
}
#endif
#endif
```

Baseline: 6.630 billion.

## Fold campaign mask kernel into fused MC stats tail to skip separate launch and sync

Adds a combined entry point that launches the campaign NaN/outlier mask kernel inside the fused quantile pipeline. It waits on a new 'done' event from the scalar-selection side stream, and it gates the mask kernel on device-side verdict and premask flags so the host does not have to read them first. It also returns the open-row count through the same readback, so the separate mask launch and the open_count .item() sync in the driver are avoided. The cost is extra event and stream coordination and more complex fallback logic, with a risk of races or deadlock if the side job fails.

```diff
diff --git a/hallthrusterpem_amd/_lib.py b/hallthrusterpem_amd/_lib.py
--- a/hallthrusterpem_amd/_lib.py
+++ b/hallthrusterpem_amd/_lib.py
@@ -81,6 +81,10 @@
     'pem_coupled_mc_stats_f64_dev': (C.c_int, [_sz, C.c_uint64, C.c_uint64, C.c_uint32, _dp, _dp, _dp, C.c_double, C.c_double, _dp, _sz,
                                                _dp, _dp, _dp, _dp, _dp, _dp, _dp, _dp, C.c_int, _dp, _dp, _dp, _dp, _dp, _dp,
                                                C.c_int, C.c_int, C.c_double, _dp, _dp, _dp, _dp]),
+    'pem_coupled_mc_campaign_f64_dev': (C.c_int, [_sz, C.c_uint64, C.c_uint64, C.c_uint32, _dp, _dp, _dp, C.c_double, C.c_double, _dp, _sz,
+                                                  _dp, _dp, _dp, _dp, _dp, _dp, _dp, _dp, C.c_int, _dp, _dp, _dp, _dp, _dp, _dp,
+                                                  C.c_int, C.c_int, C.c_double, _dp, _dp, _dp, _dp, _dp, _sz, C.c_int, _dp, _dp, C.c_int,
+                                                  _dp, _dp, _dp]),
     'pem_row_masks_f64_dev': (C.c_int, [_sz, C.c_int, _dp, _sz, _dp, _dp, _dp, _dp, _dp]),
     'pem_campaign_masks_f64_dev': (C.c_int, [_sz, C.c_int, _dp, _dp, C.c_int, C.c_int, C.c_int, C.c_double, _dp, _dp, _sz, _dp, _dp, C.c_int, _dp, _dp,
                                              C.c_int, _dp]),
diff --git a/hallthrusterpem_amd/csrc/pem_kernels.hip b/hallthrusterpem_amd/csrc/pem_kernels.hip
--- a/hallthrusterpem_amd/csrc/pem_kernels.hip
+++ b/hallthrusterpem_amd/csrc/pem_kernels.hip
@@ -2310,6 +2310,7 @@
     };
     Stage pilot, full;
     Stage side;
+    Stage done;
     std::thread worker;
     std::function<void()> body;
     bool started = false;
@@ -2321,6 +2322,7 @@
         HIP_TRY(hipEventCreateWithFlags(&pilot.ev, hipEventDisableTiming));
         HIP_TRY(hipEventCreateWithFlags(&full.ev, hipEventDisableTiming));
         HIP_TRY(hipEventCreateWithFlags(&side.ev, hipEventDisableTiming));
+        HIP_TRY(hipEventCreateWithFlags(&done.ev, hipEventDisableTiming));
         try {
             worker = std::thread(body);
         } catch (const std::exception& e) {
@@ -2332,7 +2334,7 @@
         pilot.signal(0);
         full.signal(0);
         if (worker.joinable()) worker.join();
-        for (Stage* s : {&pilot, &full, &side}) {
+        for (Stage* s : {&pilot, &full, &side, &done}) {
             if (s->ev) (void)hipEventDestroy(s->ev);
             s->ev = nullptr;
         }
@@ -2374,15 +2376,28 @@
         counted = true;
         return job ? job->full.launched(st) : PEM_OK;
     }
+    pem::CampaignMasks* masks = nullptr;
+    bool masks_launched = false;
+    int tail(const int* verdict, const int* pm_bad, int* word, hipStream_t st) override {
+        if (!masks || !job || !job->worker.joinable()) return PEM_OK;
+        if (job->done.gone.get() != 1) return PEM_OK;
+        HIP_TRY(hipStreamWaitEvent(st, job->done.ev, 0));
+        pem::CampaignMasks m = *masks;
+        if (!pm_bad) m.row_certain = m.row_uncertain = nullptr;
+        if (int rc = pem::launch_campaign_masks(m, verdict, pm_bad, st)) return rc;
+        if (m.row_certain) HIP_TRY(hipMemcpyAsync(word, m.open_count, sizeof(int32_t), hipMemcpyDeviceToDevice, st));
+        masks_launched = true;
+        return PEM_OK;
+    }
 };
 }
 
-int pem_coupled_mc_stats_f64_dev(size_t n, uint64_t first_index, uint64_t seed, uint32_t stream_id, const int32_t* kind, const double* a,
-                                 const double* b, double torr2pa, double radius, double* x_out, size_t ld, double* V_cc, double* I_B0,
-                                 double* T, double* j_ion, double* pilot_rows, double* div_angle, double* T_c, uint8_t* invalid, int nq,
-                                 const uint64_t* rank_prev, const uint64_t* rank_next, const double* gamma, double* q_out, double* q_scalars,
-                                 int* fused_ok, int q25, int q75, double iqr_factor, uint8_t* row_certain, uint8_t* row_uncertain,
-                                 int* premask_ok, pem_stream_t stream) {
+static int mc_stats_impl(size_t n, uint64_t first_index, uint64_t seed, uint32_t stream_id, const int32_t* kind, const double* a,
+                         const double* b, double torr2pa, double radius, double* x_out, size_t ld, double* V_cc, double* I_B0,
+                         double* T, double* j_ion, double* pilot_rows, double* div_angle, double* T_c, uint8_t* invalid, int nq,
+                         const uint64_t* rank_prev, const uint64_t* rank_next, const double* gamma, double* q_out, double* q_scalars,
+                         int* fused_ok, int q25, int q75, double iqr_factor, uint8_t* row_certain, uint8_t* row_uncertain,
+                         int* premask_ok, pem_stream_t stream, pem::CampaignMasks* masks, int* masks_done, int* n_open) {
     if (!kind || !a || !b || !V_cc || !div_angle || !T_c || !rank_prev || !rank_next || !gamma || !q_out || !fused_ok)
         return fail(PEM_ERR_INVALID_ARG, "pem_coupled_mc_stats: NULL array");
     if (!j_ion && !pilot_rows) return fail(PEM_ERR_INVALID_ARG, "pem_coupled_mc_stats: without a profile array, room for the pilot rows is needed");
@@ -2406,7 +2421,10 @@
         job.body = [&job, dev, side, n, nq, V_cc, qstride, rank_prev, rank_next, gamma, q_scalars]() {
             struct Release {
                 ScalarJob& j;
-                ~Release() { j.side.signal(0); }
+                ~Release() {
+                    j.side.signal(0);
+                    j.done.signal(0);
+                }
             } release{job};
             auto note = [&job](int rc) {
                 job.rc = rc;
@@ -2420,11 +2438,17 @@
             if (note(job.pilot.await(side))) return;
             pem::SidePlan plan;
             plan.ctx = &job;
+            plan.subsample_done = [](void* ctx, hipStream_t st) {
+                ScalarJob* j = static_cast<ScalarJob*>(ctx);
+                if (j->side.launched(st)) j->side.signal(0);
+                return (int)PEM_OK;
+            };
             plan.before_full = [](void* ctx, hipStream_t st) {
                 ScalarJob* j = static_cast<ScalarJob*>(ctx);
                 if (j->side.launched(st)) j->side.signal(0);
                 return j->full.await(st);
             };
+            plan.finished = [](void* ctx, hipStream_t st) { return static_cast<ScalarJob*>(ctx)->done.launched(st); };
             (void)note(pem::quantiles_side(n, 3, V_cc, 1, (size_t)qstride, nq, rank_prev, rank_next, gamma, q_scalars, side, &plan));
         };
         prod.job = &job;
@@ -2459,6 +2483,7 @@
     }
     if (premask_ok) *premask_ok = 0;
     *fused_ok = 0;
+    prod.masks = masks;
     if (int rc = pem::quantiles_fused(n, NANG, nq, rank_prev, rank_next, gamma, j_ion ? j_ion : pilot_rows, prod, q_out, fused_ok, st))
         return rc;
     if (premask_ok) *premask_ok = (*fused_ok && prod.pm_done) ? 1 : 0;
@@ -2474,7 +2499,60 @@
     if (q_scalars) {
         if (int rc = job.join()) return fail(rc, "%s", job.error.c_str());
     }
+    if (masks_done) *masks_done = (*fused_ok && prod.masks_launched) ? 1 : 0;
+    if (n_open) *n_open = (*fused_ok && prod.masks_launched) ? prod.tail_word : 0;
     return PEM_OK;
+}
+
+int pem_coupled_mc_stats_f64_dev(size_t n, uint64_t first_index, uint64_t seed, uint32_t stream_id, const int32_t* kind, const double* a,
+                                 const double* b, double torr2pa, double radius, double* x_out, size_t ld, double* V_cc, double* I_B0,
+                                 double* T, double* j_ion, double* pilot_rows, double* div_angle, double* T_c, uint8_t* invalid, int nq,
+                                 const uint64_t* rank_prev, const uint64_t* rank_next, const double* gamma, double* q_out, double* q_scalars,
+                                 int* fused_ok, int q25, int q75, double iqr_factor, uint8_t* row_certain, uint8_t* row_uncertain,
+                                 int* premask_ok, pem_stream_t stream) {
+    return mc_stats_impl(n, first_index, seed, stream_id, kind, a, b, torr2pa, radius, x_out, ld, V_cc, I_B0, T, j_ion, pilot_rows, div_angle, T_c,
+                         invalid, nq, rank_prev, rank_next, gamma, q_out, q_scalars, fused_ok, q25, q75, iqr_factor, row_certain, row_uncertain,
+                         premask_ok, stream, nullptr, nullptr, nullptr);
+}
+
+int pem_coupled_mc_campaign_f64_dev(size_t n, uint64_t first_index, uint64_t seed, uint32_t stream_id, const int32_t* kind, const double* a,
+                                    const double* b, double torr2pa, double radius, double* x_out, size_t ld, double* V_cc, double* I_B0,
+                                    double* T, double* j_ion, double* pilot_rows, double* div_angle, double* T_c, uint8_t* invalid, int nq,
+                                    const uint64_t* rank_prev, const uint64_t* rank_next, const double* gamma, double* q_out, double* q_scalars,
+                                    int* fused_ok, int q25, int q75, double iqr_factor, uint8_t* row_certain, uint8_t* row_uncertain,
+                                    int* premask_ok, uint8_t* nan_out, uint8_t* outl_out, size_t mask_ld, int thresh, int64_t* open_rows,
+                                    int32_t* open_count, int cap, int* masks_done, int* n_open, pem_stream_t stream) {
+    if (!q_scalars || !nan_out || !outl_out || !masks_done || !n_open)
+        return fail(PEM_ERR_INVALID_ARG, "pem_coupled_mc_campaign: NULL array (q_scalars, the mask arrays and the two results are required)");
+    if (q25 < 0 || q25 >= nq || q75 < 0 || q75 >= nq) return fail(PEM_ERR_INVALID_ARG, "pem_coupled_mc_campaign: q25 and q75 are rows of the nq quantiles");
+    if ((row_certain != nullptr) != (row_uncertain != nullptr) || (row_certain && (!premask_ok || !open_rows || !open_count || cap < 0)))
+        return fail(PEM_ERR_INVALID_ARG, "pem_coupled_mc_campaign: the premask counts come with premask_ok, open_rows and open_count");
+    if (mask_ld < n) return fail(PEM_ERR_INVALID_ARG, "pem_coupled_mc_campaign: rows of the mask arrays shorter than n");
+    *masks_done = 0;
+    *n_open = 0;
+    pem::CampaignMasks m;
+    m.n = n;
+    m.nvar = 3;
+    m.vars[0] = V_cc;
+    m.vars[1] = div_angle;
+    m.vars[2] = T_c;
+    m.q = q_scalars;
+    m.q_ld = 3;
+    m.row25 = q25;
+    m.row75 = q75;
+    m.iqr_factor = iqr_factor;
+    m.nan_out = nan_out;
+    m.outl_out = outl_out;
+    m.mask_ld = mask_ld;
+    m.row_certain = row_certain;
+    m.row_uncertain = row_uncertain;
+    m.thresh = thresh;
+    m.open_rows = open_rows;
+    m.open_count = open_count;
+    m.cap = cap;
+    return mc_stats_impl(n, first_index, seed, stream_id, kind, a, b, torr2pa, radius, x_out, ld, V_cc, I_B0, T, j_ion, pilot_rows, div_angle, T_c,
+                         invalid, nq, rank_prev, rank_next, gamma, q_out, q_scalars, fused_ok, q25, q75, iqr_factor, row_certain, row_uncertain,
+                         premask_ok, stream, &m, masks_done, n_open);
 }
 
 int pem_coupled_loglik_f64_dev(size_t n, double torr2pa, double radius, const double* P_b, const double* V_a,
diff --git a/hallthrusterpem_amd/csrc/pem_masks.hip b/hallthrusterpem_amd/csrc/pem_masks.hip
--- a/hallthrusterpem_amd/csrc/pem_masks.hip
+++ b/hallthrusterpem_amd/csrc/pem_masks.hip
@@ -4,6 +4,7 @@
 
 #include "pem_common.h"
 #include "pem_hip.h"
+#include "pem_qfused.h"
 
 namespace {
 
@@ -91,16 +92,19 @@
 
 namespace {
 
-constexpr int CM_MAX_VARS = 8;
+constexpr int CM_MAX_VARS = pem::CampaignMasks::MAX_VARS;
 struct CampaignVars {
     const double* v[CM_MAX_VARS];
 };
 template <int V>
 __global__ __launch_bounds__(MBLOCK) void campaign_masks_kernel(long long n, int nvar, CampaignVars vars, const double* __restrict__ q, int q_ld,
                                                                 int row25, int row75, double factor, uint8_t* __restrict__ nan_out,
-                                                                uint8_t* __restrict__ outl_out, size_t mask_ld, const uint8_t* __restrict__ certain,
+                                                                uint8_t* __restrict__ outl_out, size_t mask_ld, const uint8_t* __restrict__ certain_in,
                                                                 const uint8_t* __restrict__ uncertain, int thresh,
-                                                                long long* __restrict__ open_rows, int* __restrict__ open_count, int cap) {
+                                                                long long* __restrict__ open_rows, int* __restrict__ open_count, int cap,
+                                                                const int* __restrict__ verdict, const int* __restrict__ pm_bad) {
+    if (verdict && *verdict == 1) return;
+    const uint8_t* certain = (pm_bad && *pm_bad) ? nullptr : certain_in;
     double lo[CM_MAX_VARS], hi[CM_MAX_VARS];
 #pragma unroll
     for (int k = 0; k < CM_MAX_VARS; ++k) {
@@ -172,6 +176,30 @@
     }
 }
 
+}
+
+int pem::launch_campaign_masks(const pem::CampaignMasks& a, const int* verdict, const int* pm_bad, hipStream_t st) {
+    const size_t n = a.n;
+    const int nvar = a.nvar;
+    CampaignVars cv{};
+    for (int k = 0; k < nvar; ++k) cv.v[k] = a.vars[k];
+    int cus = 0;
+    HIP_TRY(pem::device_cus(&cus));
+    const bool words = a.mask_ld % 4 == 0 && reinterpret_cast<uintptr_t>(a.nan_out) % 4 == 0 && reinterpret_cast<uintptr_t>(a.outl_out) % 4 == 0 &&
+                       reinterpret_cast<uintptr_t>(a.row_certain) % 4 == 0 && reinterpret_cast<uintptr_t>(a.row_uncertain) % 4 == 0;
+    const int v = words ? 4 : 1;
+    long long blocks = (((long long)n + v - 1) / v + MBLOCK - 1) / MBLOCK;
+    if (blocks > (long long)cus * 16) blocks = (long long)cus * 16;
+    if (words)
+        hipLaunchKernelGGL(campaign_masks_kernel<4>, dim3((unsigned)blocks), dim3(MBLOCK), 0, st, (long long)n, nvar, cv, a.q, a.q_ld, a.row25, a.row75,
+                           a.iqr_factor, a.nan_out, a.outl_out, a.mask_ld, a.row_certain, a.row_uncertain, a.thresh, (long long*)a.open_rows,
+                           (int*)a.open_count, a.cap, verdict, pm_bad);
+    else
+        hipLaunchKernelGGL(campaign_masks_kernel<1>, dim3((unsigned)blocks), dim3(MBLOCK), 0, st, (long long)n, nvar, cv, a.q, a.q_ld, a.row25, a.row75,
+                           a.iqr_factor, a.nan_out, a.outl_out, a.mask_ld, a.row_certain, a.row_uncertain, a.thresh, (long long*)a.open_rows,
+                           (int*)a.open_count, a.cap, verdict, pm_bad);
+    HIP_TRY(hipGetLastError());
+    return PEM_OK;
 }
 
 extern "C" int pem_campaign_masks_f64_dev(size_t n, int nvar, const double* const* vars, const double* q, int q_ld, int row25, int row75,
@@ -186,27 +214,28 @@
     if (mask_ld < n) return pem::fail(PEM_ERR_INVALID_ARG, "pem_campaign_masks: rows of the mask arrays shorter than n");
     if (n == 0) return PEM_OK;
     if (int rc = pem::check_device()) return rc;
-    CampaignVars cv{};
+    pem::CampaignMasks a;
     for (int k = 0; k < nvar; ++k) {
         if (!vars[k]) return pem::fail(PEM_ERR_INVALID_ARG, "pem_campaign_masks: NULL variable");
-        cv.v[k] = vars[k];
-    }
-    int cus = 0;
-    HIP_TRY(pem::device_cus(&cus));
-    const bool words = mask_ld % 4 == 0 && reinterpret_cast<uintptr_t>(nan_out) % 4 == 0 && reinterpret_cast<uintptr_t>(outl_out) % 4 == 0 &&
-                       reinterpret_cast<uintptr_t>(row_certain) % 4 == 0 && reinterpret_cast<uintptr_t>(row_uncertain) % 4 == 0;
-    const int v = words ? 4 : 1;
-    long long blocks = (((long long)n + v - 1) / v + MBLOCK - 1) / MBLOCK;
-    if (blocks > (long long)cus * 16) blocks = (long long)cus * 16;
-    hipStream_t st = static_cast<hipStream_t>(stream);
-    if (words)
-        hipLaunchKernelGGL(campaign_masks_kernel<4>, dim3((unsigned)blocks), dim3(MBLOCK), 0, st, (long long)n, nvar, cv, q, q_ld, row25, row75, iqr_factor,
-                           nan_out, outl_out, mask_ld, row_certain, row_uncertain, thresh, (long long*)open_rows, (int*)open_count, cap);
-    else
-        hipLaunchKernelGGL(campaign_masks_kernel<1>, dim3((unsigned)blocks), dim3(MBLOCK), 0, st, (long long)n, nvar, cv, q, q_ld, row25, row75, iqr_factor,
-                           nan_out, outl_out, mask_ld, row_certain, row_uncertain, thresh, (long long*)open_rows, (int*)open_count, cap);
-    HIP_TRY(hipGetLastError());
-    return PEM_OK;
+        a.vars[k] = vars[k];
+    }
+    a.n = n;
+    a.nvar = nvar;
+    a.q = q;
+    a.q_ld = q_ld;
+    a.row25 = row25;
+    a.row75 = row75;
+    a.iqr_factor = iqr_factor;
+    a.nan_out = nan_out;
+    a.outl_out = outl_out;
+    a.mask_ld = mask_ld;
+    a.row_certain = row_certain;
+    a.row_uncertain = row_uncertain;
+    a.thresh = thresh;
+    a.open_rows = open_rows;
+    a.open_count = open_count;
+    a.cap = cap;
+    return pem::launch_campaign_masks(a, nullptr, nullptr, static_cast<hipStream_t>(stream));
 }
 
 extern "C" int pem_row_masks_f64_dev(size_t n, int m, const double* data, size_t ld, const double* lo, const double* hi, uint8_t* nan_out,
diff --git a/hallthrusterpem_amd/csrc/pem_qfused.h b/hallthrusterpem_amd/csrc/pem_qfused.h
--- a/hallthrusterpem_amd/csrc/pem_qfused.h
+++ b/hallthrusterpem_amd/csrc/pem_qfused.h
@@ -65,16 +65,42 @@
     virtual int pilot(size_t rows, double* dst, hipStream_t st) = 0;
     virtual int waves(int nq, unsigned* waves) = 0;
     virtual int count(const CountIO& io, hipStream_t st) = 0;
+    int tail_word = 0;
+    virtual int tail(const int* verdict, const int* pm_bad, int* word, hipStream_t st) {
+        (void)verdict, (void)pm_bad, (void)word, (void)st;
+        return 0;
+    }
 };
 __attribute__((visibility("hidden"))) int quantiles_fused(size_t n, int m, int nq, const uint64_t* rank_prev, const uint64_t* rank_next,
                                                           const double* gamma, double* pilot_rows, FusedProducer& prod, double* out,
                                                           int* fused_ok, hipStream_t st);
 struct SidePlan {
     int (*before_full)(void* ctx, hipStream_t st) = nullptr;
+    int (*subsample_done)(void* ctx, hipStream_t st) = nullptr;
+    int (*finished)(void* ctx, hipStream_t st) = nullptr;
     void* ctx = nullptr;
 };
 __attribute__((visibility("hidden"))) int quantiles_side(size_t n, int m, const double* data, size_t ld, size_t cs, int nq,
                                                          const uint64_t* rank_prev, const uint64_t* rank_next, const double* gamma, double* out,
                                                          hipStream_t st, const SidePlan* plan = nullptr);
 
+
+struct CampaignMasks {
+    static constexpr int MAX_VARS = 8;
+    size_t n = 0;
+    int nvar = 0;
+    const double* vars[MAX_VARS] = {};
+    const double* q = nullptr;
+    int q_ld = 0, row25 = 0, row75 = 0;
+    double iqr_factor = 0.0;
+    uint8_t *nan_out = nullptr, *outl_out = nullptr;
+    size_t mask_ld = 0;
+    const uint8_t *row_certain = nullptr, *row_uncertain = nullptr;
+    int thresh = 0;
+    int64_t* open_rows = nullptr;
+    int32_t* open_count = nullptr;
+    int cap = 0;
+};
+__attribute__((visibility("hidden"))) int launch_campaign_masks(const CampaignMasks& a, const int* verdict, const int* pm_bad, hipStream_t st);
+
 }
diff --git a/hallthrusterpem_amd/csrc/pem_quantile.hip b/hallthrusterpem_amd/csrc/pem_quantile.hip
--- a/hallthrusterpem_amd/csrc/pem_quantile.hip
+++ b/hallthrusterpem_amd/csrc/pem_quantile.hip
@@ -4,6 +4,7 @@
 #include <cmath>
 #include <cstdint>
 #include <cstdlib>
+#include <cstring>
 #include <mutex>
 
 #include "pem_common.h"
@@ -360,7 +361,9 @@
     if (lane == 0) tg[i] = T;
 }
 
-__global__ __launch_bounds__(64 * MAX_NC) void layout_kernel(int m, int nt, Target* __restrict__ tg, u64* __restrict__ total) {
+__global__ __launch_bounds__(64 * MAX_NC) void layout_kernel(int m, int nt, Target* __restrict__ tg, u64* __restrict__ total,
+                                                             const int* __restrict__ flags = nullptr, const int* __restrict__ outside = nullptr,
+                                                             u64 room = 0, int* __restrict__ verdict = nullptr) {
     __shared__ u64 start[64 * MAX_NC + 1];
     constexpr int NTMAX = 2 * PEM_QUANTILE_MAX_Q;
     const int c = threadIdx.x;
@@ -398,6 +401,7 @@
     if (c == 0) {
         for (int k = 1; k <= 64 * MAX_NC; ++k) start[k] += start[k - 1];
         total[0] = start[m];
+        if (verdict) *verdict = (flags[0] | flags[1] | flags[2] | *outside) ? 1 : (start[m] > room ? 2 : 0);
     }
     __syncthreads();
     if (c < m) {
@@ -589,7 +593,9 @@
     }
 }
 
-__global__ __launch_bounds__(QBLOCK) void select_kernel(int nt, Target* __restrict__ tg, const u64* __restrict__ cand, int* __restrict__ incomplete) {
+__global__ __launch_bounds__(QBLOCK) void select_kernel(int nt, Target* __restrict__ tg, const u64* __restrict__ cand, int* __restrict__ incomplete,
+                                                        const int* __restrict__ skip = nullptr) {
+    if (skip && *skip) return;
     Target& T = tg[blockIdx.x];
     if (T.done) return;
     if (threadIdx.x == 0 && T.owner == (int)(blockIdx.x % nt) && T.cursor != T.count && atomicExch(incomplete, 1) == 0) {
@@ -607,10 +613,10 @@
 }
 
 __global__ void finish_kernel(int m, int nq, const Column* __restrict__ col, const Target* __restrict__ tg, Wanted w,
-                              double* __restrict__ out) {
+                              double* __restrict__ out, const int* __restrict__ skip = nullptr) {
 #pragma clang fp contract(off)
     const int i = blockIdx.x * blockDim.x + threadIdx.x;
-    if (i >= m * nq) return;
+    if (i >= m * nq || (skip && *skip)) return;
     const int q = i / m, c = i - q * m;
     const double a = value_of(tg[c * 2 * nq + 2 * q].answer), b = value_of(tg[c * 2 * nq + 2 * q + 1].answer), t = w.gamma[q];
     const double diff = b - a;
@@ -921,32 +927,84 @@
     return cq;
 }
 
-constexpr int REC_UNROLL = 4;
+constexpr int REC_UNROLL = 8;
 
 constexpr int RBLOCK = 1024;
+constexpr int REC_REGIONS_LDS = 256;
+
+struct RecordWalk {
+    const pem::Record* rec;
+    const unsigned* s_cnt;
+    const unsigned* rec_count;
+    unsigned cap, waves, w, k, i0, cnt;
+    __device__ __forceinline__ unsigned count_of() const {
+        if (w >= waves) return 0u;
+        if (k < (unsigned)REC_REGIONS_LDS) return s_cnt[k];
+        const unsigned c = rec_count[w];
+        return c < cap ? c : cap;
+    }
+    __device__ __forceinline__ RecordWalk(const pem::Record* rec_, const unsigned* s_cnt_, const unsigned* rec_count_, unsigned cap_, unsigned waves_)
+        : rec(rec_), s_cnt(s_cnt_), rec_count(rec_count_), cap(cap_), waves(waves_), w(blockIdx.x), k(0), i0(0) {
+        cnt = count_of();
+    }
+    __device__ __forceinline__ void fetch(pem::Record (&e)[REC_UNROLL], unsigned& base, unsigned& n) {
+        while (w < waves && i0 >= cnt) {
+            w += gridDim.x;
+            ++k;
+            i0 = 0;
+            cnt = count_of();
+        }
+        if (w >= waves) {
+            n = 0;
+            base = 0;
+            return;
+        }
+        const pem::Record* r = rec + (size_t)w * cap;
+        base = i0 + threadIdx.x;
+        n = cnt;
+#pragma unroll
+        for (int u = 0; u < REC_UNROLL; ++u) {
+            const unsigned idx = base + u * RBLOCK;
+            e[u] = r[idx < n ? idx : 0u];
+        }
+        i0 += RBLOCK * REC_UNROLL;
+    }
+};
+__device__ __forceinline__ void record_counts_to_lds(unsigned* s_cnt, const unsigned* __restrict__ rec_count, unsigned cap, unsigned waves) {
+    for (unsigned k = threadIdx.x; k < (unsigned)REC_REGIONS_LDS; k += RBLOCK) {
+        const unsigned long long w = (unsigned long long)blockIdx.x + (unsigned long long)k * gridDim.x;
+        const unsigned c = w < waves ? rec_count[w] : 0u;
+        s_cnt[k] = c < cap ? c : cap;
+    }
+}
+
 template <int NQ>
 __global__ __launch_bounds__(RBLOCK) void record_hist_kernel(const pem::Record* __restrict__ rec, const unsigned* __restrict__ rec_count, unsigned cap,
                                                               unsigned waves, const Bracket* __restrict__ br, int lists, int bins,
                                                               unsigned* __restrict__ hist) {
     extern __shared__ unsigned lds_hist[];
     __shared__ uint4 s_br[REC_LISTS_MAX];
+    __shared__ unsigned s_cnt[REC_REGIONS_LDS];
     for (int i = threadIdx.x; i < lists * bins; i += RBLOCK) lds_hist[i] = 0;
     for (int i = threadIdx.x; i < lists; i += RBLOCK) s_br[i] = make_uint4(br[i].loh, br[i].words, br[i].mult, 0u);
-    __syncthreads();
-    for (unsigned w = blockIdx.x; w < waves; w += gridDim.x) {
-        const unsigned cnt = rec_count[w] < cap ? rec_count[w] : cap;
-        const pem::Record* r = rec + (size_t)w * cap;
-        for (unsigned i0 = threadIdx.x; i0 < cnt; i0 += RBLOCK * REC_UNROLL) {
-            pem::Record e[REC_UNROLL];
-#pragma unroll
-            for (int u = 0; u < REC_UNROLL; ++u) e[u] = r[i0 + u * RBLOCK < cnt ? i0 + u * RBLOCK : i0];
-#pragma unroll
-            for (int u = 0; u < REC_UNROLL; ++u) {
-                unsigned t, mult;
-                bool none;
-                const int cq = record_list<NQ>(s_br, e[u], t, mult, none);
-                if (!none && i0 + u * RBLOCK < cnt) atomicAdd(&lds_hist[cq * bins + (int)__umulhi(t, mult)], 1u);
-            }
+    record_counts_to_lds(s_cnt, rec_count, cap, waves);
+    __syncthreads();
+    RecordWalk walk(rec, s_cnt, rec_count, cap, waves);
+    pem::Record e[REC_UNROLL], e_next[REC_UNROLL];
+    unsigned base, n, base_next, n_next;
+    walk.fetch(e_next, base_next, n_next);
+    while (n_next) {
+#pragma unroll
+        for (int u = 0; u < REC_UNROLL; ++u) e[u] = e_next[u];
+        base = base_next;
+        n = n_next;
+        walk.fetch(e_next, base_next, n_next);
+#pragma unroll
+        for (int u = 0; u < REC_UNROLL; ++u) {
+            unsigned t, mult;
+            bool none;
+            const int cq = record_list<NQ>(s_br, e[u], t, mult, none);
+            if (!none && base + u * RBLOCK < n) atomicAdd(&lds_hist[cq * bins + (int)__umulhi(t, mult)], 1u);
         }
     }
     __syncthreads();
@@ -993,7 +1051,8 @@
 }
 
 __global__ __launch_bounds__(64) void record_offsets_kernel(int nt, int bins, const Target* __restrict__ tg, const unsigned* __restrict__ part,
-                                                             int groups, int cells, unsigned* __restrict__ woff) {
+                                                             int groups, int cells, unsigned* __restrict__ woff, const int* __restrict__ skip) {
+    if (*skip) return;
     const int i = blockIdx.x, lane = threadIdx.x, targets = gridDim.x;
     const Target T = tg[i];
     const int t = i % nt;
@@ -1017,11 +1076,13 @@
 template <int NQ>
 __global__ __launch_bounds__(RBLOCK) void record_compact_kernel(const pem::Record* __restrict__ rec, const unsigned* __restrict__ rec_count, unsigned cap,
                                                                  unsigned waves, const Bracket* __restrict__ br, int lists, Target* __restrict__ tg,
-                                                                 const unsigned* __restrict__ woff, u64* __restrict__ cand) {
+                                                                 const unsigned* __restrict__ woff, u64* __restrict__ cand, const int* __restrict__ skip) {
     __shared__ uint4 s_br[REC_LISTS_MAX];
     __shared__ int2 s_bin[REC_LISTS_MAX];
     __shared__ unsigned s_cur[2 * REC_LISTS_MAX];
     __shared__ u64 s_base[2 * REC_LISTS_MAX];
+    __shared__ unsigned s_cnt[REC_REGIONS_LDS];
+    if (*skip) return;
     const unsigned* my_off = woff + (size_t)blockIdx.x * 2 * lists;
     for (int i = threadIdx.x; i < lists; i += RBLOCK) {
         s_br[i] = make_uint4(br[i].loh, br[i].words, br[i].mult, 0u);
@@ -1032,25 +1093,28 @@
         s_base[2 * i] = T0.offset;
         s_base[2 * i + 1] = T1.offset;
     }
-    __syncthreads();
-    for (unsigned w = blockIdx.x; w < waves; w += gridDim.x) {
-        const unsigned cnt = rec_count[w] < cap ? rec_count[w] : cap;
-        const pem::Record* r = rec + (size_t)w * cap;
-        for (unsigned i0 = threadIdx.x; i0 < cnt; i0 += RBLOCK * REC_UNROLL) {
-            pem::Record e[REC_UNROLL];
-#pragma unroll
-            for (int u = 0; u < REC_UNROLL; ++u) e[u] = r[i0 + u * RBLOCK < cnt ? i0 + u * RBLOCK : i0];
-#pragma unroll
-            for (int u = 0; u < REC_UNROLL; ++u) {
-                unsigned t, mult;
-                bool none;
-                const int cq = record_list<NQ>(s_br, e[u], t, mult, none);
-                if (none || i0 + u * RBLOCK >= cnt) continue;
-                const int bin = (int)__umulhi(t, mult);
-                const int2 want = s_bin[cq];
-                const int hit = want.x == bin ? 0 : (want.y == bin ? 1 : -1);
-                if (hit >= 0) cand[s_base[2 * cq + hit] + atomicAdd(&s_cur[2 * cq + hit], 1u)] = e[u].key;
-            }
+    record_counts_to_lds(s_cnt, rec_count, cap, waves);
+    __syncthreads();
+    RecordWalk walk(rec, s_cnt, rec_count, cap, waves);
+    pem::Record e[REC_UNROLL], e_next[REC_UNROLL];
+    unsigned base, n, base_next, n_next;
+    walk.fetch(e_next, base_next, n_next);
+    while (n_next) {
+#pragma unroll
+        for (int u = 0; u < REC_UNROLL; ++u) e[u] = e_next[u];
+        base = base_next;
+        n = n_next;
+        walk.fetch(e_next, base_next, n_next);
+#pragma unroll
+        for (int u = 0; u < REC_UNROLL; ++u) {
+            unsigned t, mult;
+            bool none;
+            const int cq = record_list<NQ>(s_br, e[u], t, mult, none);
+            if (none || base + u * RBLOCK >= n) continue;
+            const int bin = (int)__umulhi(t, mult);
+            const int2 want = s_bin[cq];
+            const int hit = want.x == bin ? 0 : (want.y == bin ? 1 : -1);
+            if (hit >= 0) cand[s_base[2 * cq + hit] + atomicAdd(&s_cur[2 * cq + hit], 1u)] = e[u].key;
         }
     }
     __syncthreads();
@@ -1168,6 +1232,7 @@
     unsigned* part_buf = nullptr;
     size_t part_cap = 0;
     int ws_dev = -1;
+    u64* h_pin = nullptr;
 };
 QWork g_qwork[2];
 }
@@ -1192,6 +1257,7 @@
     const int bins1 = pow2_at_most(LDS_WORDS / m, 4096), bins2 = pow2_at_most(LDS_WORDS / (m * nt), 4096);
     int binsA = pow2_at_most((m <= 128 ? LDS_WORDS_A : LDS_WORDS) / (m * nq) - 1, 4096);
     if (fused) binsA = pow2_at_most(LDS_WORDS / (m * nq), 4096);
+    if (plan && binsA > 512) binsA = 512;
     if (const char* e = getenv("PEM_QUANTILE_BINSA")) binsA = pow2_at_most(atoll(e) < binsA ? atoll(e) : binsA, 4096);
 
     long long pilot = 32, pilot_min = 1 << 25;
@@ -1224,6 +1290,7 @@
     pem::Record*& rec_buf = work.rec_buf;
     unsigned*& part_buf = work.part_buf;
     int& ws_dev = work.ws_dev;
+    if (fused && !work.h_pin) HIP_TRY(hipHostMalloc(reinterpret_cast<void**>(&work.h_pin), 16 * sizeof(u64), hipHostMallocDefault));
     int dev = 0;
     HIP_TRY(hipGetDevice(&dev));
     if (dev != ws_dev || ws_cap < o_end) {
@@ -1264,6 +1331,8 @@
     uint4* pm_thr = reinterpret_cast<uint4*>(ws + o_pm);
     int* pm_bad = unfit + 3;
     int* inconsistent = unfit + 4;
+    int* verdict = unfit + 5;
+    int* tail_word = unfit + 6;
     Bracket* br = reinterpret_cast<Bracket*>(ws + o_br);
     u64* below = reinterpret_cast<u64*>(ws + o_bl);
     unsigned* histA = reinterpret_cast<unsigned*>(ws + o_hA);
@@ -1387,7 +1456,9 @@
     };
 
     int path = 0;
-    bool answered = false;
+    bool answered = false, read_back = false;
+    u64 h_incomplete[4] = {0, 0, 0, 0};
+    int h_inconsistent = 0;
     if (plan && !use_pilot && plan->before_full)
         if (int rc = plan->before_full(plan->ctx, st)) return cleanup(rc);
     if (use_pilot) {
@@ -1413,8 +1484,8 @@
             if (int rc = four_passes(rows_p, ld, pw, edges)) return rc;
         } else if (plan) {
             if (int rc = four_passes(rows_p, ld, pw)) return rc;
-            if (plan->before_full)
-                if (int rc = plan->before_full(plan->ctx, st)) return cleanup(rc);
+            if (plan->subsample_done)
+                if (int rc = plan->subsample_done(plan->ctx, st)) return cleanup(rc);
         } else if (int rc = four_passes(rows_p, ld * (size_t)pilot, pw)) return rc;
         const dim3 grid = grid_for(n);
         Q_TRY(hipMemsetAsync(total, 0, 256, st));
@@ -1428,6 +1499,8 @@
         unsigned rcap = 0;
         bool pm_launched = false;
         if (!fused) {
+            if (plan && plan->before_full)
+                if (int rc = plan->before_full(plan->ctx, st)) return cleanup(rc);
             Q_BY_NC(Q_BRHIST);
         } else {
             hipLaunchKernelGGL(bracket_check_kernel, dim3((unsigned)((m * nq + 63) / 64)), dim3(64), 0, st, m, nq, br, unfit);
@@ -1451,6 +1524,7 @@
                 Q_TRY(hipMalloc(&rec_buf, need * sizeof(pem::Record)));
                 rec_cap = need;
             }
+            Q_TRY(grow_candidates((u64)(4.0 * expected / (double)binsA) + 64ull * (u64)(m * nt)));
             pem::CountIO cio;
             cio.br = br;
             cio.nq = nq;
@@ -1481,7 +1555,7 @@
 #define Q_RECHIST(NQ_)                                                                                                       \
     do {                                                                                                                     \
         static pem::LdsAttrOnce attr;                                                                                        \
-        Q_TRY(attr.ensure(reinterpret_cast<const void*>(record_hist_kernel<NQ_>), 148 * 1024));  \
+        Q_TRY(attr.ensure(reinterpret_cast<const void*>(record_hist_kernel<NQ_>), 147 * 1024));  \
         hipLaunchKernelGGL(record_hist_kernel<NQ_>, dim3((unsigned)cus), dim3(RBLOCK), (size_t)m * nq * binsA * 4, st, rec_buf, rec_count, rcap, fused_waves, \
                            br, m * nq, binsA, part_buf);                                                                     \
     } while (0)
@@ -1500,33 +1574,20 @@
             hipLaunchKernelGGL(record_total_check_kernel, dim3(1), dim3(64), 0, st, rec_sums, inconsistent, prod_flags);
         }
         hipLaunchKernelGGL(decide_bracket_kernel, dim3((unsigned)(m * nt)), dim3(64), 0, st, nt, col, br, below, histA, binsA, tg, outside);
-        hipLaunchKernelGGL(layout_kernel, dim3(1), dim3(64 * MAX_NC), 0, st, m, nt, tg, total);
-        Q_TRY(hipGetLastError());
         u64 h_tot[2] = {0, 0};
-        int h_unfit4[4] = {0, 0, 0, 0};
-        Q_TRY(hipMemcpyAsync(h_tot, total, 2 * sizeof(u64), hipMemcpyDeviceToHost, st));
-        if (fused) Q_TRY(hipMemcpyAsync(h_unfit4, unfit, sizeof h_unfit4, hipMemcpyDeviceToHost, st));
-        Q_TRY(hipStreamSynchronize(st));
-        if (fused) fused->pm_done = (pm_launched && h_unfit4[3] == 0) ? 1 : 0;
-        if (fused && (h_unfit4[0] || (int)(h_tot[1] & 0xffffffffull) != 0 || h_unfit4[1] || h_unfit4[2])) {
-            *fused_ok = 0;
-            return cleanup(PEM_OK);
-        }
-        if ((int)(h_tot[1] & 0xffffffffull) == 0) {
-            Q_TRY(grow_candidates(h_tot[0]));
-            u64* cand = cand_buf;
-#define Q_BRCOMPACT_(NC_, NQ_) \
-    hipLaunchKernelGGL((compact_bracket_kernel<NC_, NQ_>), grid, blk, 0, st, (long long)n, m, ld, cs, data, br, tg, cand)
-#define Q_BRCOMPACT(NC_) Q_BY_NQ_##NC_(Q_BRCOMPACT_, NC_)
-            if (!fused) {
-                Q_BY_NC(Q_BRCOMPACT);
-            } else {
-                int cus = 256;
-                Q_TRY(pem::device_cus(&cus));
-                unsigned* woff = part_buf + (size_t)cus * m * nq * binsA;
-                hipLaunchKernelGGL(record_offsets_kernel, dim3((unsigned)(m * nt)), dim3(64), 0, st, nt, binsA, tg, part_buf, cus, m * nq * binsA, woff);
+        if (fused) {
+            int cus = 256;
+            Q_TRY(pem::device_cus(&cus));
+            unsigned* woff = part_buf + (size_t)cus * m * nq * binsA;
+            u64 room = cand_cap - 1;
+            if (const char* e = getenv("PEM_QUANTILE_CAND_ROOM")) room = (u64)atoll(e) < room ? (u64)atoll(e) : room;
+            bool tail_done = false, room_grown = false;
+            for (int attempt = 0;; ++attempt) {
+                u64* cand = cand_buf;
+                hipLaunchKernelGGL(layout_kernel, dim3(1), dim3(64 * MAX_NC), 0, st, m, nt, tg, total, unfit, outside, room, verdict);
+                hipLaunchKernelGGL(record_offsets_kernel, dim3((unsigned)(m * nt)), dim3(64), 0, st, nt, binsA, tg, part_buf, cus, m * nq * binsA, woff, verdict);
 #define Q_RECCOMPACT(NQ_) \
-    hipLaunchKernelGGL(record_compact_kernel<NQ_>, dim3((unsigned)cus), dim3(RBLOCK), 0, st, rec_buf, rec_count, rcap, fused_waves, br, m * nq, tg, woff, cand)
+    hipLaunchKernelGGL(record_compact_kernel<NQ_>, dim3((unsigned)cus), dim3(RBLOCK), 0, st, rec_buf, rec_count, rcap, fused_waves, br, m * nq, tg, woff, cand, verdict)
                 switch (nq) {
                     case 1: Q_RECCOMPACT(1); break;
                     case 2: Q_RECCOMPACT(2); break;
@@ -1536,7 +1597,50 @@
                     default: Q_RECCOMPACT(6); break;
                 }
 #undef Q_RECCOMPACT
-            }
+                hipLaunchKernelGGL(select_kernel, dim3((unsigned)(m * nt)), blk, 0, st, nt, tg, cand, incomplete, verdict);
+                hipLaunchKernelGGL(finish_kernel, dim3((unsigned)((m * nq + 63) / 64)), dim3(64), 0, st, m, nq, col, tg, w, out, verdict);
+                Q_TRY(hipGetLastError());
+                if (!tail_done)
+                    if (int rc = fused->tail(verdict, pm_launched ? pm_bad : nullptr, tail_word, st)) return cleanup(rc);
+                tail_done = true;
+                u64* h_blk = work.h_pin;
+                Q_TRY(hipMemcpyAsync(h_blk, total, 13 * sizeof(u64), hipMemcpyDeviceToHost, st));
+                Q_TRY(hipStreamSynchronize(st));
+                int h_flags[7];
+                memcpy(h_flags, reinterpret_cast<const char*>(h_blk) + 72, sizeof h_flags);
+                fused->tail_word = h_flags[6];
+                h_tot[0] = h_blk[0];
+                h_tot[1] = h_blk[1];
+                memcpy(h_incomplete, h_blk + 2, sizeof h_incomplete);
+                h_inconsistent = h_flags[4];
+                fused->pm_done = (pm_launched && h_flags[3] == 0) ? 1 : 0;
+                const bool declined = h_flags[0] || (int)(h_tot[1] & 0xffffffffull) != 0 || h_flags[1] || h_flags[2];
+                if (declined) {
+                    *fused_ok = 0;
+                    return cleanup(PEM_OK);
+                }
+                if (h_flags[5] == 0) break;
+                if (h_flags[5] != 2 || attempt > 0)
+                    return pem::fail(PEM_ERR_HIP, "pem_quantiles: the device's verdict on the fused tail (%d) contradicts its flags (internal error; result discarded)", h_flags[5]);
+                Q_TRY(grow_candidates(h_tot[0]));
+                room = cand_cap - 1;
+                room_grown = true;
+            }
+            answered = true;
+            path = room_grown ? 3 : 1;
+            read_back = true;
+        } else {
+        hipLaunchKernelGGL(layout_kernel, dim3(1), dim3(64 * MAX_NC), 0, st, m, nt, tg, total);
+        Q_TRY(hipGetLastError());
+        Q_TRY(hipMemcpyAsync(h_tot, total, 2 * sizeof(u64), hipMemcpyDeviceToHost, st));
+        Q_TRY(hipStreamSynchronize(st));
+        if ((int)(h_tot[1] & 0xffffffffull) == 0) {
+            Q_TRY(grow_candidates(h_tot[0]));
+            u64* cand = cand_buf;
+#define Q_BRCOMPACT_(NC_, NQ_) \
+    hipLaunchKernelGGL((compact_bracket_kernel<NC_, NQ_>), grid, blk, 0, st, (long long)n, m, ld, cs, data, br, tg, cand)
+#define Q_BRCOMPACT(NC_) Q_BY_NQ_##NC_(Q_BRCOMPACT_, NC_)
+            Q_BY_NC(Q_BRCOMPACT);
             hipLaunchKernelGGL(select_kernel, dim3((unsigned)(m * nt)), blk, 0, st, nt, tg, cand, incomplete);
             Q_TRY(hipGetLastError());
             answered = true;
@@ -1544,16 +1648,19 @@
         } else {
             path = 2;
         }
-    }
-    if (!answered)
-        if (int rc = four_passes(n, ld, w)) return rc;
-    hipLaunchKernelGGL(finish_kernel, dim3((unsigned)((m * nq + 63) / 64)), dim3(64), 0, st, m, nq, col, tg, w, out);
-    Q_TRY(hipGetLastError());
-    u64 h_incomplete[4] = {0, 0, 0, 0};
-    int h_inconsistent = 0;
-    Q_TRY(hipMemcpyAsync(h_incomplete, incomplete, sizeof h_incomplete, hipMemcpyDeviceToHost, st));
-    Q_TRY(hipMemcpyAsync(&h_inconsistent, inconsistent, sizeof(int), hipMemcpyDeviceToHost, st));
-    Q_TRY(hipStreamSynchronize(st));
+        }
+    }
+    if (!read_back) {
+        if (!answered)
+            if (int rc = four_passes(n, ld, w)) return rc;
+        hipLaunchKernelGGL(finish_kernel, dim3((unsigned)((m * nq + 63) / 64)), dim3(64), 0, st, m, nq, col, tg, w, out);
+        Q_TRY(hipGetLastError());
+        if (plan && plan->finished)
+            if (int rc = plan->finished(plan->ctx, st)) return cleanup(rc);
+        Q_TRY(hipMemcpyAsync(h_incomplete, incomplete, sizeof h_incomplete, hipMemcpyDeviceToHost, st));
+        Q_TRY(hipMemcpyAsync(&h_inconsistent, inconsistent, sizeof(int), hipMemcpyDeviceToHost, st));
+        Q_TRY(hipStreamSynchronize(st));
+    }
     if (h_inconsistent > 0)
         return pem::fail(PEM_ERR_HIP, "pem_quantiles: the histogram of column %d does not add up to its number of values (internal error; result discarded; path %d)",
                          h_inconsistent - 1, path);
diff --git a/hallthrusterpem_amd/drivers.py b/hallthrusterpem_amd/drivers.py
--- a/hallthrusterpem_amd/drivers.py
+++ b/hallthrusterpem_amd/drivers.py
@@ -257,6 +257,7 @@
     batch = CoupledBatch(n, device=device, profile=keep_profile)
     pct = [25.0, 75.0] + [float(x) for x in percentiles]
     answered, premasked, qj, qs, certain, uncertain = False, False, None, None, None, None
+    masked, n_open = False, 0
     thresh = int(0.75 * _lib.NANGLE)
     nv, cap = len(QOI_NAMES), 65536
     dev = batch.device
@@ -276,17 +277,19 @@
             pilot = None if keep_profile else torch.empty(((n + 31) // 32, _lib.NANGLE), dtype=torch.float64, device=dev)
             certain = torch.empty(n, dtype=torch.uint8, device=dev)
             uncertain = torch.empty(n, dtype=torch.uint8, device=dev)
-            ok, pm_ok = C.c_int(0), C.c_int(0)
+            ok, pm_ok, m_ok, m_open = C.c_int(0), C.c_int(0), C.c_int(0), C.c_int(0)
             ptr = lambda arr: C.c_void_p(arr.ctypes.data)
             outs = batch._out_ptrs
-            _lib.check(_lib.load().pem_coupled_mc_stats_f64_dev(
+            _lib.check(_lib.load().pem_coupled_mc_campaign_f64_dev(
                 n, 0, design.seed, design.stream, ptr(design.kind), ptr(design.a), ptr(design.b), constants.TORR_2_PA, batch.radius,
                 C.c_void_p(batch.inputs.data_ptr()) if keep_inputs else None, batch.inputs.stride(0),
                 outs[0], outs[1], outs[2], outs[3], None if pilot is None else C.c_void_p(pilot.data_ptr()), outs[4], outs[5], outs[6],
                 len(pct), ptr(rp), ptr(rn), ptr(gm), C.c_void_p(qj.data_ptr()), C.c_void_p(qs.data_ptr()), C.byref(ok),
                 0, 1, float(iqr_factor), C.c_void_p(certain.data_ptr()), C.c_void_p(uncertain.data_ptr()), C.byref(pm_ok),
-                C.c_void_p(stream.cuda_stream)))
+                C.c_void_p(nan_s.data_ptr()), C.c_void_p(out_s.data_ptr()), nan_s.stride(0), thresh, C.c_void_p(open_rows.data_ptr()),
+                C.c_void_p(open_count.data_ptr()), cap, C.byref(m_ok), C.byref(m_open), C.c_void_p(stream.cuda_stream)))
             answered, premasked = bool(ok.value), bool(pm_ok.value)
+            masked, n_open = bool(m_ok.value), int(m_open.value)
             del pilot
         else:
             batch.run_mc(design, first_index=0, write_inputs=keep_inputs)
@@ -311,10 +314,12 @@
     nan_idx, outlier_idx, bands = {}, {}, {}
     dp = lambda t: C.c_void_p(t.data_ptr())
     with torch.cuda.device(dev):
-        vars_ = (C.c_void_p * nv)(*[batch.qoi[i].data_ptr() for i in range(nv)])
-        _lib.check(_lib.load().pem_campaign_masks_f64_dev(
-            n, nv, vars_, dp(qs), qs.stride(0), 0, 1, float(iqr_factor), dp(nan_s), dp(out_s), nan_s.stride(0), dp(certain) if premasked else None,
-            dp(uncertain) if premasked else None, thresh, dp(open_rows), dp(open_count), cap, C.c_void_p(torch.cuda.current_stream(dev).cuda_stream)))
+        if not masked:
+            vars_ = (C.c_void_p * nv)(*[batch.qoi[i].data_ptr() for i in range(nv)])
+            _lib.check(_lib.load().pem_campaign_masks_f64_dev(
+                n, nv, vars_, dp(qs), qs.stride(0), 0, 1, float(iqr_factor), dp(nan_s), dp(out_s), nan_s.stride(0),
+                dp(certain) if premasked else None, dp(uncertain) if premasked else None, thresh, dp(open_rows), dp(open_count), cap,
+                C.c_void_p(torch.cuda.current_stream(dev).cuda_stream)))
     for i, k in enumerate(QOI_NAMES):
         nan_idx[k], outlier_idx[k] = nan_s[i], out_s[i]
 
@@ -322,7 +327,8 @@
         iqr = qj[1] - qj[0]
         return qj[0] - iqr_factor * iqr, qj[1] + iqr_factor * iqr
     if premasked:
-        n_open = int(open_count.item())
+        if not masked:
+            n_open = int(open_count.item())
         if n_open > cap:
             c, u = certain.to(torch.int32), uncertain.to(torch.int32)
             rows_open = torch.nonzero((c <= thresh) & (c + u > thresh)).flatten()
diff --git a/include/pem_hip.h b/include/pem_hip.h
--- a/include/pem_hip.h
+++ b/include/pem_hip.h
@@ -204,6 +204,13 @@
                                  const uint64_t* rank_prev, const uint64_t* rank_next, const double* gamma, double* q_out, double* q_scalars,
                                  int* fused_ok, int q25, int q75, double iqr_factor, uint8_t* row_certain, uint8_t* row_uncertain,
                                  int* premask_ok, pem_stream_t stream);
+int pem_coupled_mc_campaign_f64_dev(size_t n, uint64_t first_index, uint64_t seed, uint32_t stream_id, const int32_t* kind, const double* a,
+                                    const double* b, double torr2pa, double radius, double* x_out, size_t ld, double* V_cc, double* I_B0,
+                                    double* T, double* j_ion, double* pilot_rows, double* div_angle, double* T_c, uint8_t* invalid, int nq,
+                                    const uint64_t* rank_prev, const uint64_t* rank_next, const double* gamma, double* q_out, double* q_scalars,
+                                    int* fused_ok, int q25, int q75, double iqr_factor, uint8_t* row_certain, uint8_t* row_uncertain,
+                                    int* premask_ok, uint8_t* nan_out, uint8_t* outl_out, size_t mask_ld, int thresh, int64_t* open_rows,
+                                    int32_t* open_count, int cap, int* masks_done, int* n_open, pem_stream_t stream);
 
 #define PEM_ROW_MASKS_MAX_M 512
 int pem_row_masks_f64_dev(size_t n, int m, const double* data, size_t ld, const double* lo, const double* hi, uint8_t* nan_out,
```

Result: no change. 6.667 billion (median of 5 runs) (+0.6%).
